# ai-forever/Kandinsky-2

Measured on NVIDIA H100. Metric: unet_denoising_steps_per_sec, higher is better.
Workload: dtype f16

## Files before the change

kandinsky-2_b200/csrc/k2_api.cu:

```cuda
#include <stdio.h>
#include <stdlib.h>
#include <string.h>

#include <algorithm>
#include <atomic>
#include <mutex>

#include "../../include/k2b200.h"
#include "k2_internal.h"

namespace k2 {

static thread_local std::string g_err;
static std::atomic<long long> g_launches{0};
static int g_force_bn = 0;
static int g_force_split = 0;
static int g_pdl = 0;


void set_error(const std::string& msg) { g_err = msg; }
int fail(const std::string& msg) {
  g_err = msg;
  return -1;
}
void count_launch(int n) { g_launches.fetch_add(n, std::memory_order_relaxed); }

bool pdl_enabled() { return g_pdl != 0; }
static int g_conv_epi_sets = 1;
static int g_gn_bps = 0;
int gn_apply_blocks_per_sm() { return g_gn_bps; }

int num_sms() {
  static int n = 0;
  if (n == 0) {
    int dev = 0;
    cudaGetDevice(&dev);
    cudaDeviceGetAttribute(&n, cudaDevAttrMultiProcessorCount, dev);
    if (n <= 0) n = 132;
  }
  return n;
}

typedef CUresult (*EncodeTiledFn)(CUtensorMap*, CUtensorMapDataType, cuuint32_t, void*, const cuuint64_t*,
                                  const cuuint64_t*, const cuuint32_t*, const cuuint32_t*,
                                  CUtensorMapInterleave, CUtensorMapSwizzle, CUtensorMapL2promotion,
                                  CUtensorMapFloatOOBfill);

static EncodeTiledFn get_encode_fn() {
  static EncodeTiledFn fn = nullptr;
  static std::once_flag once;
  std::call_once(once, [] {
    void* p = nullptr;
    cudaDriverEntryPointQueryResult qres;
    cudaError_t e = cudaGetDriverEntryPoint("cuTensorMapEncodeTiled", &p, cudaEnableDefault, &qres);
    if (e == cudaSuccess && qres == cudaDriverEntryPointSuccess) fn = reinterpret_cast<EncodeTiledFn>(p);
  });
  return fn;
}

int encode_tmap_f16(CUtensorMap* out, const void* base, int rank, const uint64_t* dims,
                    const uint64_t* strides_bytes, const uint32_t* box) {
  EncodeTiledFn fn = get_encode_fn();
  if (!fn) return fail("cuTensorMapEncodeTiled unavailable (no CUDA driver)");
  cuuint64_t gdim[5];
  cuuint64_t gstr[4];
  cuuint32_t bx[5];
  cuuint32_t es[5];
  for (int i = 0; i < rank; ++i) {
    gdim[i] = dims[i];
    bx[i] = box[i];
    es[i] = 1;
  }
  for (int i = 0; i + 1 < rank; ++i) gstr[i] = strides_bytes[i];
  CUresult r = fn(out, CU_TENSOR_MAP_DATA_TYPE_FLOAT16, static_cast<cuuint32_t>(rank), const_cast<void*>(base),
                  gdim, gstr, bx, es, CU_TENSOR_MAP_INTERLEAVE_NONE, CU_TENSOR_MAP_SWIZZLE_128B,
                  CU_TENSOR_MAP_L2_PROMOTION_L2_256B, CU_TENSOR_MAP_FLOAT_OOB_FILL_NONE);
  if (r != CUDA_SUCCESS) {
    char buf[256];
    snprintf(buf, sizeof buf,
             "cuTensorMapEncodeTiled failed (%d): rank %d dims %llu %llu %llu %llu box %u %u %u %u base %p",
             static_cast<int>(r), rank, (unsigned long long)dims[0], (unsigned long long)(rank > 1 ? dims[1] : 0),
             (unsigned long long)(rank > 2 ? dims[2] : 0), (unsigned long long)(rank > 3 ? dims[3] : 0), box[0],
             rank > 1 ? box[1] : 0, rank > 2 ? box[2] : 0, rank > 3 ? box[3] : 0, base);
    return fail(buf);
  }
  return 0;
}

static void choose_tile(int NB, int H, int W, int& TN, int& TH, int& TW, bool single_image_only = false) {
  long long best_tiles[2] = {-1, -1};
  int bn[2] = {1, 1}, bw[2] = {1, 1}, bh[2] = {1, 1};
  const int wmax = W < 128 ? W : 128;
  for (int tw = 1; tw <= wmax; ++tw) {
    const long long tiles_w = (W + tw - 1) / tw;
    for (int tn = 1; tn <= NB && tn * tw <= 128; ++tn) {
      int thmax = 128 / (tw * tn);
      if (thmax > H) thmax = H;
      if (thmax < 1) continue;
      const long long tiles_h = (H + thmax - 1) / thmax;
      const int th = static_cast<int>((H + tiles_h - 1) / tiles_h);
      const long long tiles = tiles_h * tiles_w * ((NB + tn - 1) / tn);
      for (int k = (tn == 1 ? 0 : 1); k < 2; ++k) {
        bool better = best_tiles[k] < 0 || tiles < best_tiles[k];
        if (!better && tiles == best_tiles[k]) {
          if (tn != bn[k]) {
            better = tn < bn[k];
          } else {
            const int d_new = tw > th ? tw - th : th - tw;
            const int d_old = bw[k] > bh[k] ? bw[k] - bh[k] : bh[k] - bw[k];
            better = (d_new < d_old) || (d_new == d_old && tw > bw[k]);
          }
        }
        if (better) {
          best_tiles[k] = tiles;
          bn[k] = tn;
          bw[k] = tw;
          bh[k] = th;
        }
      }
    }
  }
  const int k = (!single_image_only && best_tiles[1] * 100 <= best_tiles[0] * 85) ? 1 : 0;
  TN = bn[k];
  TW = bw[k];
  TH = bh[k];
}


struct ConvPlan {
  int TN, TH, TW, tiles_w, tiles_h, tiles_n, m_tiles;
  int m_tiles_phase;
  int BN, splits;
  int fuse_stats, row_groups;
  int es;
};

static void plan_conv(int NB, int H, int W, bool any9, int kchunks, int Cout, int out_mode, bool has_workspace,
                      long long workspace_bytes, bool want_gn, ConvPlan& pl, const int* cfg = nullptr, bool up2 = false,
                      bool w_batched = false) {
  const int g_force_bn = (cfg && cfg[0]) ? cfg[0] : k2::g_force_bn;
  const int g_force_split = (cfg && cfg[2]) ? cfg[2] : k2::g_force_split;
  pl.es = (cfg && cfg[3]) ? cfg[3] : k2::g_conv_epi_sets;
  choose_tile(NB, H, W, pl.TN, pl.TH, pl.TW, w_batched);
  pl.tiles_w = (W + pl.TW - 1) / pl.TW;
  pl.tiles_h = (H + pl.TH - 1) / pl.TH;
  pl.tiles_n = (NB + pl.TN - 1) / pl.TN;
  pl.m_tiles = pl.tiles_w * pl.tiles_h * pl.tiles_n;
  pl.m_tiles_phase = pl.m_tiles;

  int BN = g_force_bn;
  int splits = 1;
  const long long M_total = static_cast<long long>(NB) * H * W;
  const bool can_split = !up2 && !w_batched && has_workspace && out_mode == 0 && Cout % 8 == 0;
  auto split_ok = [&](int sp) {
    if (sp == 1) return true;
    const int kps = (kchunks + sp - 1) / sp;
    return can_split && kps >= 8 && (sp - 1) * kps < kchunks &&
           static_cast<long long>(sp) * M_total * Cout * 4 <= workspace_bytes;
  };
  auto model = [&](int bn, int sp) {
    const long long nt = (Cout + bn - 1) / bn;
    const long long units = static_cast<long long>(pl.m_tiles) * nt * sp * (up2 ? 4 : 1);
    const long long slots = num_sms();
    const long long waves = (units + slots - 1) / slots;
    const long long kps = (kchunks + sp - 1) / sp;
    long long cost = waves * (kps * (4LL * bn + 60) + 2000);
    if (sp > 1) cost += 4000 + (static_cast<long long>(sp) + 1) * M_total * Cout * 4 / 1800;
    return cost;
  };
  if (BN == 0) {
    if (Cout <= 16) BN = 16;
    else if (Cout <= 64) BN = 64;
    else if (Cout <= 128) BN = 128;
    else BN = 0;
  }
  {
    const int cand[3] = {256, 192, 128};
    long long best = -1;
    int best_bn = BN ? BN : 256, best_sp = 1;
    for (int ci = 0; ci < 3; ++ci) {
      const int bn = BN ? BN : cand[ci];
      if (BN && ci > 0) break;
      for (int sp = 1; sp <= 8; ++sp) {
        if (g_force_split > 0 && sp != g_force_split) continue;
        if (!split_ok(sp)) continue;
        const long long c = model(bn, sp);
        if (best < 0 || c < best) {
          best = c;
          best_bn = bn;
          best_sp = sp;
        }
      }
    }
    BN = best_bn;
    splits = best_sp;
  }
  pl.BN = BN;
  pl.splits = splits;

  pl.fuse_stats = 0;
  pl.row_groups = 0;
  if (want_gn && out_mode == 0 && Cout % 8 == 0) {
    if (splits == 1 && BN >= 64 && Cout % 64 == 0 && (pl.TN == 1 || pl.TH * pl.TW == 16)) {
      pl.fuse_stats = 1;
      pl.row_groups = ((pl.TN == 1) ? pl.m_tiles : NB * pl.tiles_h * pl.tiles_w) * (up2 ? 4 : 1);
    } else if (splits > 1 && (static_cast<long long>(H) * W) % 16 == 0) {
      pl.fuse_stats = 2;
      pl.row_groups = static_cast<int>(M_total / 16);
    }
  }
}

static void plan_to_info(const ConvPlan& pl, int* info) {
  if (!info) return;
  info[0] = pl.BN; info[1] = 0;
  info[2] = pl.splits; info[3] = pl.m_tiles; info[4] = pl.TN;
  info[5] = pl.fuse_stats; info[6] = pl.row_groups;
}

}

using namespace k2;

extern "C" {

const char* k2_last_error(void) { return g_err.c_str(); }
int k2_version(void) { return 100; }
long long k2_launch_count(void) { return g_launches.load(); }
void k2_reset_launch_count(void) { g_launches.store(0); }
int k2_set_tuning(int key, int value) {
  if (key == 0) {
    g_force_bn = value;
    return 0;
  }
  if (key == 1) {
    g_force_split = value;
    return 0;
  }
  if (key == 2) {
    if (value == 2) return fail("k2_set_tuning: no CTA-pair conv kernel on sm_90");
    return 0;
  }
  if (key == 4) {
    g_pdl = value;
    return 0;
  }
  if (key == 10) {
    g_conv_epi_sets = (value == 2) ? 2 : 1;
    return 0;
  }
  if (key == 11) {
    g_gn_bps = value;
    return 0;
  }
  if (key == 9) {
    return 0;
  }

  return fail("k2_set_tuning: unknown key");
}

int k2_conv_gemm(const K2ConvSrc* srcs, int nsrc, int NB, int H, int W, const void* w_packed, int w_rows,
                 int Ktot, int ldw, int Cout, const float* bias, const void* residual, int ldr, void* out, int ldo,
                 int out_mode, void* workspace, long long workspace_bytes, float* gn_partial, int* info,
                 k2_stream_t stream) {
  return k2_conv_gemm_cfg(srcs, nsrc, NB, H, W, w_packed, w_rows, Ktot, ldw, Cout, bias, residual, ldr, out, ldo, out_mode,
                          workspace, workspace_bytes, gn_partial, info, nullptr, 0, stream);
}

int k2_conv_gemm_cfg(const K2ConvSrc* srcs, int nsrc, int NB, int H, int W, const void* w_packed, int w_rows,
                     int Ktot, int ldw, int Cout, const float* bias, const void* residual, int ldr, void* out, int ldo,
                     int out_mode, void* workspace, long long workspace_bytes, float* gn_partial, int* info,
                     const int* cfg, long long w_batch_stride, k2_stream_t stream) {
  K2_REQUIRE(w_batch_stride >= 0 && w_batch_stride % 8 == 0, "conv_gemm_cfg: w_batch_stride must be a multiple of 8 elements");
  K2_REQUIRE(out_mode == 0 || out_mode == 1, "conv_gemm: out_mode must be 0 (fp16 rows) or 1 (fp32 NCHW)");
  K2_REQUIRE(out_mode == 0 || residual == nullptr, "conv_gemm: out_mode 1 (fp32 NCHW) takes no residual");
  const bool w_batched = w_batch_stride > 0;
  if (cfg) {
    K2_REQUIRE(cfg[0] == 0 || cfg[0] == 16 || cfg[0] == 64 || cfg[0] == 128 || cfg[0] == 192 || cfg[0] == 256,
               "conv_gemm_cfg: N tile must be 0, 16, 64, 128, 192 or 256");
    K2_REQUIRE(cfg[1] >= 0 && cfg[1] <= 2 && cfg[2] >= 0 && cfg[2] <= 8 && cfg[3] >= 0 && cfg[3] <= 2,
               "conv_gemm_cfg: pair mode in 0..2, splits in 0..8, epilogue sets in 0..2");
    K2_REQUIRE(cfg[1] != 2, "conv_gemm_cfg: no CTA-pair conv kernel on sm_90");
  }
  K2_REQUIRE(nsrc >= 1 && nsrc <= 3, "conv_gemm: 1..3 sources");
  K2_REQUIRE((reinterpret_cast<uintptr_t>(gn_partial) & 7) == 0, "conv_gemm: gn_partial must be 8-byte aligned");
  K2_REQUIRE(NB > 0 && H > 0 && W > 0 && Cout > 0, "conv_gemm: bad geometry");
  K2_REQUIRE(w_rows >= Cout, "conv_gemm: w_rows < Cout");
  K2_REQUIRE(Ktot % 64 == 0, "conv_gemm: Ktot must be a multiple of 64");
  if (ldw == 0) ldw = Ktot;
  K2_REQUIRE(ldw >= Ktot && ldw % 8 == 0 && (reinterpret_cast<uintptr_t>(w_packed) & 15) == 0,
             "conv_gemm: weight row stride / alignment");
  ConvGemmParams p;
  memset(&p, 0, sizeof p);
  p.NB = NB;
  p.H = H;
  p.W = W;
  bool any9 = false;
  int kchunks = 0;
  const bool up2 = srcs[0].taps == 4;
  if (up2) {
    K2_REQUIRE(nsrc == 1 && out_mode == 0 && residual == nullptr && H % 2 == 0 && W % 2 == 0,
               "conv_gemm: a taps == 4 source (3x3 conv over its nearest-2x upsampling) must be the only source, with fp16 "
               "output, no residual and even output H, W");
    H /= 2;
    W /= 2;
    p.H = H;
    p.W = W;
  }
  for (int s = 0; s < nsrc; ++s) {
    const K2ConvSrc& src = srcs[s];
    K2_REQUIRE(src.taps == 9 || src.taps == 1 || (s == 0 && src.taps == 4), "conv_gemm: taps must be 9 or 1 (or 4: up2)");
    K2_REQUIRE(src.C > 0 && src.C % 8 == 0 && src.ld % 8 == 0 && src.ld >= src.C, "conv_gemm: bad source C/ld");
    K2_REQUIRE((reinterpret_cast<uintptr_t>(src.ptr) & 15) == 0, "conv_gemm: source not 16B aligned");
    any9 = any9 || src.taps == 9;
    p.seg_taps[s] = src.taps;
    p.seg_kchunks[s] = (src.C + 63) / 64;
    kchunks += src.taps * p.seg_kchunks[s];
  }
  K2_REQUIRE(kchunks * 64 * (up2 ? 4 : 1) == Ktot,
             "conv_gemm: Ktot does not match the sources (taps * ceil(C/64)*64 summed; x4 phases for a taps == 4 source)");
  p.num_k_chunks = kchunks;

  ConvPlan pl;
  plan_conv(NB, H, W, any9 || up2, kchunks, Cout, out_mode, workspace != nullptr, workspace_bytes, gn_partial != nullptr, pl,
            cfg, up2, w_batched);
  K2_REQUIRE(!w_batched || (!up2 && pl.TN == 1), "conv_gemm_cfg: batched weights need single-image tiles");
  p.w_batched = w_batched ? 1 : 0;
  plan_to_info(pl, info);
  p.TN = pl.TN;
  p.TH = pl.TH;
  p.TW = pl.TW;
  p.tiles_w = pl.tiles_w;
  p.tiles_h = pl.tiles_h;
  p.tiles_n = pl.tiles_n;
  p.m_tiles = up2 ? 4 * pl.m_tiles_phase : pl.m_tiles;
  p.m_tiles_phase = pl.m_tiles_phase;
  p.up2 = up2 ? 1 : 0;
  p.a_box_bytes = static_cast<uint32_t>(p.TN * p.TH * p.TW * 128);
  for (int s = 0; s < nsrc; ++s) {
    const K2ConvSrc& src = srcs[s];
    uint64_t dims[4] = {static_cast<uint64_t>(src.C), static_cast<uint64_t>(W), static_cast<uint64_t>(H),
                        static_cast<uint64_t>(NB)};
    uint64_t str[3] = {static_cast<uint64_t>(src.ld) * 2, static_cast<uint64_t>(src.ld) * 2 * W,
                       static_cast<uint64_t>(src.ld) * 2 * W * H};
    uint32_t box[4] = {64, static_cast<uint32_t>(p.TW), static_cast<uint32_t>(p.TH), static_cast<uint32_t>(p.TN)};
    if (encode_tmap_f16(&p.tmA[s], src.ptr, 4, dims, str, box)) return -1;
  }
  const int BN = pl.BN, splits = pl.splits, fuse_stats = pl.fuse_stats;
  p.splits = splits;
  p.k_per_split = (kchunks + splits - 1) / splits;
  p.M_total = static_cast<long long>(NB) * H * W * (up2 ? 4 : 1);
  p.ws = reinterpret_cast<float*>(workspace);
  p.n_tiles = (Cout + BN - 1) / BN;
  p.Cout = Cout;
  {
    uint64_t dims[3] = {static_cast<uint64_t>(Ktot), static_cast<uint64_t>(w_rows), static_cast<uint64_t>(w_batched ? NB : 1)};
    uint64_t str[2] = {static_cast<uint64_t>(ldw) * 2,
                       (w_batched ? static_cast<uint64_t>(w_batch_stride) : static_cast<uint64_t>(ldw) * w_rows) * 2};
    uint32_t box[3] = {64, static_cast<uint32_t>(BN), 1};
    if (encode_tmap_f16(&p.tmB, w_packed, 3, dims, str, box)) return -1;
  }
  p.bias = bias;
  p.residual = reinterpret_cast<const __half*>(residual);
  p.ldr = ldr;
  p.out = out;
  p.ldo = ldo;
  p.out_mode = (splits > 1) ? 2 : out_mode;
  p.gn_part = (fuse_stats == 1) ? reinterpret_cast<float2*>(gn_partial) : nullptr;
  p.gn_mode = (fuse_stats == 1) ? (p.TN == 1 ? 1 : 2) : 0;
  if (out_mode == 0) {
    K2_REQUIRE(ldo % 8 == 0 && (reinterpret_cast<uintptr_t>(out) & 15) == 0, "conv_gemm: out alignment");
    if (residual)
      K2_REQUIRE(ldr % 8 == 0 && (reinterpret_cast<uintptr_t>(residual) & 15) == 0, "conv_gemm: residual alignment");
  }
  int rc = launch_conv_gemm(p, BN, pl.es, static_cast<cudaStream_t>(stream));
  if (rc == 0) g_launches.fetch_add(1, std::memory_order_relaxed);
  if (rc == 0 && splits > 1) {
    rc = launch_splitk_finalize(p.ws, splits, p.M_total, Cout, bias, p.residual, ldr, reinterpret_cast<__half*>(out), ldo,
                                fuse_stats == 2 ? reinterpret_cast<float2*>(gn_partial) : nullptr,
                                static_cast<cudaStream_t>(stream));
    if (rc == 0) g_launches.fetch_add(1, std::memory_order_relaxed);
  }
  return rc;
}

int k2_conv_plan(int NB, int H, int W, int taps, int Ktot, int Cout, int out_mode, long long workspace_bytes,
                 int want_gn_partial, int* info) {
  K2_REQUIRE(NB > 0 && H > 0 && W > 0 && Cout > 0 && info, "conv_plan: bad arguments");
  K2_REQUIRE(Ktot > 0 && Ktot % 64 == 0, "conv_plan: Ktot must be a positive multiple of 64");
  ConvPlan pl;
  plan_conv(NB, H, W, taps == 9, Ktot / 64, Cout, out_mode, workspace_bytes > 0, workspace_bytes, want_gn_partial != 0, pl);
  plan_to_info(pl, info);
  return 0;
}

}
```

kandinsky-2_b200/csrc/k2_common.cuh:

```cuda
#pragma once
#include <cuda.h>
#include <cuda_fp16.h>
#include <cuda_runtime.h>
#include <stdint.h>
#include <stdio.h>

namespace k2 {

__device__ __forceinline__ uint32_t smem_u32(const void* p) {
  return static_cast<uint32_t>(__cvta_generic_to_shared(p));
}

__device__ __forceinline__ uint32_t lane_id() { return threadIdx.x & 31; }

__device__ __forceinline__ bool elect_one() {
  uint32_t pred = 0;
  asm volatile(
      "{\n"
      ".reg .b32 rx;\n"
      ".reg .pred px;\n"
      "elect.sync rx|px, 0xffffffff;\n"
      "selp.b32 %0, 1, 0, px;\n"
      "}\n"
      : "=r"(pred));
  return pred != 0;
}

__device__ __forceinline__ void mbar_init(uint64_t* bar, uint32_t count) {
  asm volatile("mbarrier.init.shared::cta.b64 [%0], %1;" ::"r"(smem_u32(bar)), "r"(count));
}
__device__ __forceinline__ void fence_barrier_init() {
  asm volatile("fence.mbarrier_init.release.cluster;" ::: "memory");
}
__device__ __forceinline__ void mbar_arrive_expect_tx(uint64_t* bar, uint32_t bytes) {
  asm volatile("mbarrier.arrive.expect_tx.shared::cta.b64 _, [%0], %1;" ::"r"(smem_u32(bar)),
               "r"(bytes)
               : "memory");
}
__device__ __forceinline__ void mbar_arrive(uint64_t* bar) {
  asm volatile("mbarrier.arrive.shared::cta.b64 _, [%0];" ::"r"(smem_u32(bar)) : "memory");
}
__device__ __forceinline__ bool mbar_try_wait(uint64_t* bar, uint32_t parity) {
  uint32_t ok;
  asm volatile(
      "{\n"
      ".reg .pred p;\n"
      "mbarrier.try_wait.parity.shared::cta.b64 p, [%1], %2;\n"
      "selp.b32 %0, 1, 0, p;\n"
      "}\n"
      : "=r"(ok)
      : "r"(smem_u32(bar)), "r"(parity)
      : "memory");
  return ok != 0;
}
__device__ __forceinline__ void mbar_wait(uint64_t* bar, uint32_t parity) {
  if (mbar_try_wait(bar, parity)) return;
  long long t0 = clock64();
  while (!mbar_try_wait(bar, parity)) {
    if (clock64() - t0 > 4000000000LL) {
      printf("k2b200: mbarrier wait timeout (block %d,%d,%d thread %d)\n", blockIdx.x, blockIdx.y,
             blockIdx.z, threadIdx.x);
      __trap();
    }
  }
}

__device__ __forceinline__ void mbar_wait_lean(uint64_t* bar, uint32_t parity) {
  if (mbar_try_wait(bar, parity)) return;
  long long t0 = clock64();
  while (!mbar_try_wait(bar, parity)) {
    if (clock64() - t0 > 4000000000LL) __trap();
  }
}

__device__ __forceinline__ void fence_proxy_async_smem() {
  asm volatile("fence.proxy.async.shared::cta;" ::: "memory");
}

__device__ __forceinline__ void tma_prefetch_desc(const CUtensorMap* tm) {
  asm volatile("prefetch.tensormap [%0];" ::"l"(reinterpret_cast<uint64_t>(tm)) : "memory");
}
__device__ __forceinline__ void tma_load_2d(void* dst, const CUtensorMap* tm, uint64_t* bar, int c0,
                                            int c1) {
  asm volatile(
      "cp.async.bulk.tensor.2d.shared::cluster.global.mbarrier::complete_tx::bytes [%0], [%1, {%3, "
      "%4}], [%2];"
      ::"r"(smem_u32(dst)),
      "l"(reinterpret_cast<uint64_t>(tm)), "r"(smem_u32(bar)), "r"(c0), "r"(c1)
      : "memory");
}
__device__ __forceinline__ void tma_load_3d(void* dst, const CUtensorMap* tm, uint64_t* bar, int c0,
                                            int c1, int c2) {
  asm volatile(
      "cp.async.bulk.tensor.3d.shared::cluster.global.mbarrier::complete_tx::bytes [%0], [%1, {%3, "
      "%4, %5}], [%2];"
      ::"r"(smem_u32(dst)),
      "l"(reinterpret_cast<uint64_t>(tm)), "r"(smem_u32(bar)), "r"(c0), "r"(c1), "r"(c2)
      : "memory");
}
__device__ __forceinline__ void tma_load_4d(void* dst, const CUtensorMap* tm, uint64_t* bar, int c0,
                                            int c1, int c2, int c3) {
  asm volatile(
      "cp.async.bulk.tensor.4d.shared::cluster.global.mbarrier::complete_tx::bytes [%0], [%1, {%3, "
      "%4, %5, %6}], [%2];"
      ::"r"(smem_u32(dst)),
      "l"(reinterpret_cast<uint64_t>(tm)), "r"(smem_u32(bar)), "r"(c0), "r"(c1), "r"(c2), "r"(c3)
      : "memory");
}

__device__ __forceinline__ uint64_t make_wgmma_desc(uint32_t smem_addr) {
  uint64_t d = 0;
  d |= static_cast<uint64_t>((smem_addr & 0x3FFFF) >> 4);
  d |= static_cast<uint64_t>(1) << 16;
  d |= static_cast<uint64_t>(1024 >> 4) << 32;
  d |= static_cast<uint64_t>(1) << 62;
  return d;
}
__device__ __forceinline__ void wgmma_fence() { asm volatile("wgmma.fence.sync.aligned;" ::: "memory"); }
__device__ __forceinline__ void wgmma_commit() { asm volatile("wgmma.commit_group.sync.aligned;" ::: "memory"); }
template <int N>
__device__ __forceinline__ void wgmma_wait() {
  asm volatile("wgmma.wait_group.sync.aligned %0;" ::"n"(N) : "memory");
}
__device__ __forceinline__ void wgmma_m64n16k16(float (&d)[8], uint64_t adesc, uint64_t bdesc, uint32_t accumulate) {
  asm volatile(
      "{\n"
      ".reg .pred p;\n"
      "setp.ne.b32 p, %10, 0;\n"
      "wgmma.mma_async.sync.aligned.m64n16k16.f32.f16.f16 "
      "{%0, %1, %2, %3, %4, %5, %6, %7}, %8, %9, p, 1, 1, 0, 0;\n"
      "}\n"
      : "+f"(d[0]), "+f"(d[1]), "+f"(d[2]), "+f"(d[3]), "+f"(d[4]), "+f"(d[5]), "+f"(d[6]), "+f"(d[7])
      : "l"(adesc), "l"(bdesc), "r"(accumulate));
}

__device__ __forceinline__ void wgmma_m64n64k16(float (&d)[32], uint64_t adesc, uint64_t bdesc, uint32_t accumulate) {
  asm volatile(
      "{\n"
      ".reg .pred p;\n"
      "setp.ne.b32 p, %34, 0;\n"
      "wgmma.mma_async.sync.aligned.m64n64k16.f32.f16.f16 "
      "{%0, %1, %2, %3, %4, %5, %6, %7, %8, %9, %10, %11, %12, %13, %14, %15, %16, %17, %18, %19, %20, %21, %22, %23, %24, %25, %26, %27, %28, %29, %30, %31}, %32, %33, p, 1, 1, 0, 0;\n"
      "}\n"
      : "+f"(d[0]), "+f"(d[1]), "+f"(d[2]), "+f"(d[3]), "+f"(d[4]), "+f"(d[5]), "+f"(d[6]), "+f"(d[7]), "+f"(d[8]), "+f"(d[9]), "+f"(d[10]), "+f"(d[11]), "+f"(d[12]), "+f"(d[13]), "+f"(d[14]), "+f"(d[15]), "+f"(d[16]), "+f"(d[17]), "+f"(d[18]), "+f"(d[19]), "+f"(d[20]), "+f"(d[21]), "+f"(d[22]), "+f"(d[23]), "+f"(d[24]), "+f"(d[25]), "+f"(d[26]), "+f"(d[27]), "+f"(d[28]), "+f"(d[29]), "+f"(d[30]), "+f"(d[31])
      : "l"(adesc), "l"(bdesc), "r"(accumulate));
}

#define K2_WGMMA_D8(o)                                                                                                  \
  "+f"(d[(o)]), "+f"(d[(o) + 1]), "+f"(d[(o) + 2]), "+f"(d[(o) + 3]), "+f"(d[(o) + 4]), "+f"(d[(o) + 5]), "+f"(d[(o) + 6]), \
      "+f"(d[(o) + 7])
#define K2_WGMMA_D32(o) K2_WGMMA_D8(o), K2_WGMMA_D8((o) + 8), K2_WGMMA_D8((o) + 16), K2_WGMMA_D8((o) + 24)

__device__ __forceinline__ void wgmma_m64n128k16(float (&d)[64], uint64_t adesc, uint64_t bdesc, uint32_t accumulate) {
  asm volatile(
      "{\n"
      ".reg .pred p;\n"
      "setp.ne.b32 p, %66, 0;\n"
      "wgmma.mma_async.sync.aligned.m64n128k16.f32.f16.f16 {"
      "%0, %1, %2, %3, %4, %5, %6, %7, %8, %9, %10, %11, %12, %13, %14, %15, "
      "%16, %17, %18, %19, %20, %21, %22, %23, %24, %25, %26, %27, %28, %29, %30, %31, "
      "%32, %33, %34, %35, %36, %37, %38, %39, %40, %41, %42, %43, %44, %45, %46, %47, "
      "%48, %49, %50, %51, %52, %53, %54, %55, %56, %57, %58, %59, %60, %61, %62, %63"
      "}, %64, %65, p, 1, 1, 0, 0;\n"
      "}\n"
      : K2_WGMMA_D32(0), K2_WGMMA_D32(32)
      : "l"(adesc), "l"(bdesc), "r"(accumulate));
}

__device__ __forceinline__ void wgmma_m64n192k16(float (&d)[96], uint64_t adesc, uint64_t bdesc, uint32_t accumulate) {
  asm volatile(
      "{\n"
      ".reg .pred p;\n"
      "setp.ne.b32 p, %98, 0;\n"
      "wgmma.mma_async.sync.aligned.m64n192k16.f32.f16.f16 {"
      "%0, %1, %2, %3, %4, %5, %6, %7, %8, %9, %10, %11, %12, %13, %14, %15, "
      "%16, %17, %18, %19, %20, %21, %22, %23, %24, %25, %26, %27, %28, %29, %30, %31, "
      "%32, %33, %34, %35, %36, %37, %38, %39, %40, %41, %42, %43, %44, %45, %46, %47, "
      "%48, %49, %50, %51, %52, %53, %54, %55, %56, %57, %58, %59, %60, %61, %62, %63, "
      "%64, %65, %66, %67, %68, %69, %70, %71, %72, %73, %74, %75, %76, %77, %78, %79, "
      "%80, %81, %82, %83, %84, %85, %86, %87, %88, %89, %90, %91, %92, %93, %94, %95"
      "}, %96, %97, p, 1, 1, 0, 0;\n"
      "}\n"
      : K2_WGMMA_D32(0), K2_WGMMA_D32(32), K2_WGMMA_D32(64)
      : "l"(adesc), "l"(bdesc), "r"(accumulate));
}

__device__ __forceinline__ void wgmma_m64n256k16(float (&d)[128], uint64_t adesc, uint64_t bdesc, uint32_t accumulate) {
  asm volatile(
      "{\n"
      ".reg .pred p;\n"
      "setp.ne.b32 p, %130, 0;\n"
      "wgmma.mma_async.sync.aligned.m64n256k16.f32.f16.f16 {"
      "%0, %1, %2, %3, %4, %5, %6, %7, %8, %9, %10, %11, %12, %13, %14, %15, "
      "%16, %17, %18, %19, %20, %21, %22, %23, %24, %25, %26, %27, %28, %29, %30, %31, "
      "%32, %33, %34, %35, %36, %37, %38, %39, %40, %41, %42, %43, %44, %45, %46, %47, "
      "%48, %49, %50, %51, %52, %53, %54, %55, %56, %57, %58, %59, %60, %61, %62, %63, "
      "%64, %65, %66, %67, %68, %69, %70, %71, %72, %73, %74, %75, %76, %77, %78, %79, "
      "%80, %81, %82, %83, %84, %85, %86, %87, %88, %89, %90, %91, %92, %93, %94, %95, "
      "%96, %97, %98, %99, %100, %101, %102, %103, %104, %105, %106, %107, %108, %109, %110, %111, "
      "%112, %113, %114, %115, %116, %117, %118, %119, %120, %121, %122, %123, %124, %125, %126, %127"
      "}, %128, %129, p, 1, 1, 0, 0;\n"
      "}\n"
      : K2_WGMMA_D32(0), K2_WGMMA_D32(32), K2_WGMMA_D32(64), K2_WGMMA_D32(96)
      : "l"(adesc), "l"(bdesc), "r"(accumulate));
}
__device__ __forceinline__ uint64_t make_wgmma_desc_mn(uint32_t smem_addr) {
  uint64_t d = 0;
  d |= static_cast<uint64_t>((smem_addr & 0x3FFFF) >> 4);
  d |= static_cast<uint64_t>(1) << 16;
  d |= static_cast<uint64_t>(1024 >> 4) << 32;
  d |= static_cast<uint64_t>(1) << 62;
  return d;
}

__device__ __forceinline__ void wgmma_m64n64k16_rs_tb(float (&d)[32], const uint32_t (&a)[4], uint64_t bdesc) {
  asm volatile(
      "{\n"
      "wgmma.mma_async.sync.aligned.m64n64k16.f32.f16.f16 {"
      "%0, %1, %2, %3, %4, %5, %6, %7, %8, %9, %10, %11, %12, %13, %14, %15, "
      "%16, %17, %18, %19, %20, %21, %22, %23, %24, %25, %26, %27, %28, %29, %30, %31"
      "}, {%32, %33, %34, %35}, %36, 1, 1, 1, 1;\n"
      "}\n"
      : K2_WGMMA_D32(0)
      : "r"(a[0]), "r"(a[1]), "r"(a[2]), "r"(a[3]), "l"(bdesc));
}
#undef K2_WGMMA_D32
#undef K2_WGMMA_D8

__device__ __forceinline__ void reg_fence(float& r) { asm volatile("" : "+f"(r)::"memory"); }

template <int R>
__device__ __forceinline__ void setmaxnreg_dec() {
  asm volatile("setmaxnreg.dec.sync.aligned.u32 %0;" ::"n"(R));
}
template <int R>
__device__ __forceinline__ void setmaxnreg_inc() {
  asm volatile("setmaxnreg.inc.sync.aligned.u32 %0;" ::"n"(R));
}

__device__ __forceinline__ void mma_16816(float (&d)[4], const uint32_t (&a)[4], uint32_t b0, uint32_t b1) {
  asm volatile(
      "mma.sync.aligned.m16n8k16.row.col.f32.f16.f16.f32 {%0, %1, %2, %3}, {%4, %5, %6, %7}, {%8, %9}, "
      "{%0, %1, %2, %3};"
      : "+f"(d[0]), "+f"(d[1]), "+f"(d[2]), "+f"(d[3])
      : "r"(a[0]), "r"(a[1]), "r"(a[2]), "r"(a[3]), "r"(b0), "r"(b1));
}
__device__ __forceinline__ void ldmatrix_x4(uint32_t (&r)[4], uint32_t saddr) {
  asm volatile("ldmatrix.sync.aligned.m8n8.x4.shared.b16 {%0, %1, %2, %3}, [%4];"
               : "=r"(r[0]), "=r"(r[1]), "=r"(r[2]), "=r"(r[3])
               : "r"(saddr));
}
__device__ __forceinline__ void ldmatrix_x4_trans(uint32_t (&r)[4], uint32_t saddr) {
  asm volatile("ldmatrix.sync.aligned.m8n8.x4.trans.shared.b16 {%0, %1, %2, %3}, [%4];"
               : "=r"(r[0]), "=r"(r[1]), "=r"(r[2]), "=r"(r[3])
               : "r"(saddr));
}
__device__ __forceinline__ void cp_async_16(uint32_t saddr, const void* gptr, int src_bytes) {
  asm volatile("cp.async.cg.shared.global [%0], [%1], 16, %2;" ::"r"(saddr), "l"(gptr), "r"(src_bytes) : "memory");
}
__device__ __forceinline__ void cp_async_commit() { asm volatile("cp.async.commit_group;" ::: "memory"); }
template <int N>
__device__ __forceinline__ void cp_async_wait() {
  asm volatile("cp.async.wait_group %0;" ::"n"(N) : "memory");
}

__device__ __forceinline__ void sts_v4(uint32_t saddr, uint32_t a, uint32_t b, uint32_t c, uint32_t d) {
  asm volatile("st.shared.v4.b32 [%0], {%1, %2, %3, %4};" ::"r"(saddr), "r"(a), "r"(b), "r"(c), "r"(d) : "memory");
}
__device__ __forceinline__ uint4 lds_v4(uint32_t saddr) {
  uint4 v;
  asm volatile("ld.shared.v4.b32 {%0, %1, %2, %3}, [%4];" : "=r"(v.x), "=r"(v.y), "=r"(v.z), "=r"(v.w) : "r"(saddr) : "memory");
  return v;
}
__device__ __forceinline__ uint32_t lds_u32(uint32_t saddr) {
  uint32_t v;
  asm volatile("ld.shared.b32 %0, [%1];" : "=r"(v) : "r"(saddr) : "memory");
  return v;
}
__device__ __forceinline__ void named_bar_sync(int id, int count) {
  asm volatile("bar.sync %0, %1;" ::"r"(id), "r"(count) : "memory");
}
__device__ __forceinline__ void named_bar_arrive(int id, int count) {
  asm volatile("bar.arrive %0, %1;" ::"r"(id), "r"(count) : "memory");
}
__device__ __forceinline__ void pdl_wait() { asm volatile("griddepcontrol.wait;" ::: "memory"); }
__device__ __forceinline__ void pdl_launch() { asm volatile("griddepcontrol.launch_dependents;" ::: "memory"); }

__device__ __forceinline__ float silu_f(float x) {
  float e, r;
  asm("ex2.approx.ftz.f32 %0, %1;" : "=f"(e) : "f"(-1.44269504088896341f * x));
  asm("rcp.approx.ftz.f32 %0, %1;" : "=f"(r) : "f"(1.f + e));
  return x * r;
}

}
```

kandinsky-2_b200/csrc/k2_conv_gemm.cu:

```cuda
#include <stdio.h>

#include "k2_common.cuh"
#include "k2_internal.h"

namespace k2 {

namespace {

constexpr int BM = 128;
constexpr int BK = 64;
constexpr int A_STAGE_BYTES = BM * BK * 2;
constexpr int ACC_PAD = 4;

constexpr int EPI_STAGE_FLOATS = 32 * 33;
constexpr int EPI_BYTES = 4 * EPI_STAGE_FLOATS * 4 + 4 * 256 * 4;
constexpr int SMEM_LIMIT = 227 * 1024;

template <int BN, int ES>
struct Cfg {
  static constexpr int B_STAGE_BYTES = BN * BK * 2;
  static constexpr int STAGE_BYTES = A_STAGE_BYTES + B_STAGE_BYTES;
  static constexpr int BNC = (BN < 64) ? BN : (ES == 2 ? 128 : 64);
  static_assert(ES == 1 || BN % 128 == 0, "two epilogue sets need N tiles of 128 or 256");
  static constexpr int ACC_BYTES = BM * (BNC + ACC_PAD) * 4;
  static constexpr int BAR_BYTES = 256;
  static constexpr int FIXED = ACC_BYTES + ES * EPI_BYTES + BAR_BYTES + 1024;
  static constexpr int STAGES = (SMEM_LIMIT - FIXED) / STAGE_BYTES > 6 ? 6 : (SMEM_LIMIT - FIXED) / STAGE_BYTES;
  static constexpr int SMEM_BYTES = STAGES * STAGE_BYTES + FIXED;
  static_assert(STAGES >= 2, "conv_gemm: shared memory does not hold two pipeline stages");
};

__device__ __forceinline__ void decode_m_tile(const ConvGemmParams& p, int m_idx, int& n0, int& y0,
                                              int& x0, int& phase) {
  phase = 0;
  if (p.up2) {
    phase = m_idx / p.m_tiles_phase;
    m_idx -= phase * p.m_tiles_phase;
  }
  int tw_i = m_idx % p.tiles_w;
  int t = m_idx / p.tiles_w;
  int th_i = t % p.tiles_h;
  int tn_i = t / p.tiles_h;
  x0 = tw_i * p.TW;
  y0 = th_i * p.TH;
  n0 = tn_i * p.TN;
}

template <int N>
__device__ __forceinline__ void acc_ld(const float* src, uint32_t (&r)[N]) {
#pragma unroll
  for (int v = 0; v < N / 4; ++v) {
    const float4 t = *reinterpret_cast<const float4*>(src + 4 * v);
    r[4 * v] = __float_as_uint(t.x);
    r[4 * v + 1] = __float_as_uint(t.y);
    r[4 * v + 2] = __float_as_uint(t.z);
    r[4 * v + 3] = __float_as_uint(t.w);
  }
}

template <int BN, int ES>
__device__ __forceinline__ void epilogue_tile(const ConvGemmParams& p, const float* acc, int ew, int lane, int n0, int y0,
                                              int x0, int cbase, int split, int m_idx, float* stat_smem, int es_arg,
                                              int phase) {
  const int es = (ES == 1) ? 0 : es_arg;
  const int row = ew * 32 + lane;
  const int thw = p.TH * p.TW;
  constexpr int CH = (BN >= 32) ? 32 : 16;
  const float* arow = acc + row * (BN + ACC_PAD);
      const int tn = row / thw;
      const int rem = row - tn * thw;
      const int th = rem / p.TW;
      const int tw = rem - th * p.TW;
      const int n = n0 + tn, y = y0 + th, x = x0 + tw;
      const bool valid = (tn < p.TN) && (n < p.NB) && (y < p.H) && (x < p.W);
      const long long out_row = p.up2 ? (static_cast<long long>(n) * (2 * p.H) + (2 * y + (phase >> 1))) * (2 * p.W) + (2 * x + (phase & 1))
                                      : (static_cast<long long>(n) * p.H + y) * p.W + x;
      const int m_in = p.up2 ? m_idx - phase * p.m_tiles_phase : m_idx;
      auto part_index = [&](long long base) { return p.up2 ? base * 4 + phase : base; };
      if constexpr (BN % 64 == 0) {
        if ((p.out_mode == 0 && p.Cout % 64 == 0) || (p.out_mode == 2 && p.Cout % 32 == 0)) {
          const uint32_t stage = smem_u32(stat_smem + (es * 4 + ew) * EPI_STAGE_FLOATS);
          float* bsm = stat_smem + 4 * ES * EPI_STAGE_FLOATS + (es * 4 + ew) * 256;
          const int my_pix = valid ? static_cast<int>(out_row) : -1;
          const int sub = lane >> 3, piece = lane & 7;
          int pix[8];
#pragma unroll
          for (int i = 0; i < 8; ++i) pix[i] = __shfl_sync(0xffffffffu, my_pix, i * 4 + sub);
          const uint32_t own = stage + lane * 128;
          if (p.out_mode == 2) {
            float* wsb = p.ws + static_cast<long long>(split) * p.M_total * p.Cout;
#pragma unroll 1
            for (int j = 0; j < BN / 32; ++j) {
              const int col0 = cbase + j * 32;
              if (col0 >= p.Cout) break;
              if constexpr (ES > 1) {
                if ((j % ES) != es) continue;
              }
              uint32_t r[32];
              acc_ld(arow + j * 32, r);
#pragma unroll
              for (int v = 0; v < 8; ++v)
                sts_v4(own + ((v ^ (lane & 7)) << 4), r[v * 4], r[v * 4 + 1], r[v * 4 + 2], r[v * 4 + 3]);
              __syncwarp();
#pragma unroll
              for (int i = 0; i < 8; ++i) {
                const int rr = i * 4 + sub;
                const uint4 v4 = lds_v4(stage + rr * 128 + ((piece ^ (rr & 7)) << 4));
                if (pix[i] >= 0)
                  *reinterpret_cast<uint4*>(wsb + static_cast<long long>(pix[i]) * p.Cout + col0 + piece * 4) = v4;
              }
              __syncwarp();
            }
            return;
          }
          constexpr int NP = BN / 64;
          if (p.bias) {
#pragma unroll
            for (int c = lane; c < BN; c += 32) bsm[c] = (cbase + c < p.Cout) ? __ldg(p.bias + cbase + c) : 0.f;
            __syncwarp();
          }
          __half* outb = reinterpret_cast<__half*>(p.out);
          float4 st[NP];
          uint4 rpre[8];
          auto load_res = [&](int jp) {
            const int c0 = cbase + jp * 64;
#pragma unroll
            for (int i = 0; i < 8; ++i) {
              rpre[i] = make_uint4(0u, 0u, 0u, 0u);
              if (pix[i] >= 0 && c0 < p.Cout)
                rpre[i] = *reinterpret_cast<const uint4*>(p.residual + static_cast<long long>(pix[i]) * p.ldr + c0 + piece * 8);
            }
          };
          if constexpr (ES == 1) {
            if (p.residual) load_res(0);
          }
#pragma unroll
          for (int jp = 0; jp < NP; ++jp) {
            const int col0 = cbase + jp * 64;
            st[jp] = make_float4(0.f, 0.f, 0.f, 0.f);
            if (col0 < p.Cout && (ES == 1 || (jp % ES) == es)) {
              if constexpr (ES > 1) {
                if (p.residual) load_res(jp);
              }
              if (p.residual) {
#pragma unroll
                for (int i = 0; i < 8; ++i) {
                  const int rr = i * 4 + sub;
                  sts_v4(stage + rr * 128 + ((piece ^ (rr & 7)) << 4), rpre[i].x, rpre[i].y, rpre[i].z, rpre[i].w);
                }
                __syncwarp();
              }
              if constexpr (ES == 1) {
                if (p.residual && jp + 1 < NP) load_res(jp + 1);
              }
#pragma unroll
              for (int v = 0; v < 8; ++v) {
                uint32_t r[8];
                acc_ld(arow + jp * 64 + v * 8, r);
                float f[8];
#pragma unroll
                for (int e = 0; e < 8; ++e) f[e] = __uint_as_float(r[e]);
                if (p.bias) {
                  const float4 b0 = *reinterpret_cast<const float4*>(bsm + jp * 64 + v * 8);
                  const float4 b1 = *reinterpret_cast<const float4*>(bsm + jp * 64 + v * 8 + 4);
                  f[0] += b0.x; f[1] += b0.y; f[2] += b0.z; f[3] += b0.w;
                  f[4] += b1.x; f[5] += b1.y; f[6] += b1.z; f[7] += b1.w;
                }
                const uint32_t slot = own + ((v ^ (lane & 7)) << 4);
                if (p.residual) {
                  const uint4 rv = lds_v4(slot);
                  const __half2* rh = reinterpret_cast<const __half2*>(&rv);
#pragma unroll
                  for (int e = 0; e < 4; ++e) {
                    const float2 t = __half22float2(rh[e]);
                    f[2 * e] += t.x;
                    f[2 * e + 1] += t.y;
                  }
                }
                uint32_t o[4];
#pragma unroll
                for (int e = 0; e < 4; ++e) {
                  const __half2 hh = __floats2half2_rn(f[2 * e], f[2 * e + 1]);
                  o[e] = valid ? *reinterpret_cast<const uint32_t*>(&hh) : 0u;
                }
                sts_v4(slot, o[0], o[1], o[2], o[3]);
              }
              __syncwarp();
#pragma unroll
              for (int i = 0; i < 8; ++i) {
                const int rr = i * 4 + sub;
                const uint4 v4 = lds_v4(stage + rr * 128 + ((piece ^ (rr & 7)) << 4));
                if (pix[i] >= 0)
                  *reinterpret_cast<uint4*>(outb + static_cast<long long>(pix[i]) * p.ldo + col0 + piece * 8) = v4;
              }
              if (p.gn_part) {
                float4 h0 = make_float4(0.f, 0.f, 0.f, 0.f), h1 = make_float4(0.f, 0.f, 0.f, 0.f);
#pragma unroll
                for (int rr = 0; rr < 32; ++rr) {
                  const uint32_t w = lds_u32(stage + rr * 128 + (((lane >> 2) ^ (rr & 7)) << 4) + ((lane & 3) << 2));
                  const float2 t = __half22float2(*reinterpret_cast<const __half2*>(&w));
                  float4& hacc = (rr < 16) ? h0 : h1;
                  hacc.x += t.x;
                  hacc.y = fmaf(t.x, t.x, hacc.y);
                  hacc.z += t.y;
                  hacc.w = fmaf(t.y, t.y, hacc.w);
                }
                if (p.gn_mode == 2) {
                  const int per = p.tiles_h * p.tiles_w;
                  const int sp = m_in % per;
                  const int img = n0 + 2 * ew;
                  if (2 * ew < p.TN && img < p.NB)
                    *reinterpret_cast<float4*>(p.gn_part + part_index(static_cast<long long>(img) * per + sp) * p.Cout + col0 + 2 * lane) = h0;
                  if (2 * ew + 1 < p.TN && img + 1 < p.NB)
                    *reinterpret_cast<float4*>(p.gn_part + part_index(static_cast<long long>(img + 1) * per + sp) * p.Cout + col0 + 2 * lane) = h1;
                } else {
                  st[jp] = make_float4(h0.x + h1.x, h0.y + h1.y, h0.z + h1.z, h0.w + h1.w);
                }
              }
              __syncwarp();
            }
          }
          if (p.gn_part && p.gn_mode == 1) {
            if constexpr (ES == 1) {
              float4* mine = reinterpret_cast<float4*>(stat_smem + ew * EPI_STAGE_FLOATS);
#pragma unroll
              for (int jp = 0; jp < NP; ++jp) mine[jp * 32 + lane] = st[jp];
              named_bar_sync(1, 128);
              if (ew < NP) {
                const int col0 = cbase + ew * 64;
                if (col0 < p.Cout) {
                  float4 acc = make_float4(0.f, 0.f, 0.f, 0.f);
#pragma unroll
                  for (int w = 0; w < 4; ++w) {
                    const float4 t = reinterpret_cast<const float4*>(stat_smem + w * EPI_STAGE_FLOATS)[ew * 32 + lane];
                    acc.x += t.x; acc.y += t.y; acc.z += t.z; acc.w += t.w;
                  }
                  *reinterpret_cast<float4*>(p.gn_part + part_index(m_in) * p.Cout + col0 + 2 * lane) = acc;
                }
              }
              named_bar_sync(1, 128);
            } else {
              float4* mine = reinterpret_cast<float4*>(stat_smem + (es * 4 + ew) * EPI_STAGE_FLOATS);
#pragma unroll
              for (int jp = 0; jp < NP; ++jp) mine[jp * 32 + lane] = st[jp];
              named_bar_sync(1 + es, 128);
              const int jp_f = es + ew * ES;
              if (jp_f < NP) {
                const int col0 = cbase + jp_f * 64;
                if (col0 < p.Cout) {
                  float4 acc = make_float4(0.f, 0.f, 0.f, 0.f);
#pragma unroll
                  for (int w = 0; w < 4; ++w) {
                    const float4 t =
                        reinterpret_cast<const float4*>(stat_smem + (es * 4 + w) * EPI_STAGE_FLOATS)[jp_f * 32 + lane];
                    acc.x += t.x; acc.y += t.y; acc.z += t.z; acc.w += t.w;
                  }
                  *reinterpret_cast<float4*>(p.gn_part + part_index(m_in) * p.Cout + col0 + 2 * lane) = acc;
                }
              }
              named_bar_sync(1 + es, 128);
            }
          }
          return;
        }
      }
#pragma unroll 1
      for (int j = 0; j < BN / CH; ++j) {
        uint32_t r[CH];
        acc_ld(arow + j * CH, r);
        const int col0 = cbase + j * CH;
        if (valid && col0 < p.Cout) {
          if (p.out_mode == 2) {
            float* w = p.ws + (static_cast<long long>(split) * p.M_total + out_row) * p.Cout + col0;
            if (col0 + CH <= p.Cout) {
#pragma unroll
              for (int v = 0; v < CH / 4; ++v)
                *reinterpret_cast<uint4*>(w + v * 4) = make_uint4(r[v * 4], r[v * 4 + 1], r[v * 4 + 2], r[v * 4 + 3]);
            } else {
#pragma unroll
              for (int e = 0; e < CH; ++e)
                if (col0 + e < p.Cout) w[e] = __uint_as_float(r[e]);
            }
          } else if (p.out_mode == 0) {
            __half* orow = reinterpret_cast<__half*>(p.out) + out_row * p.ldo + col0;
            const __half* rrow = p.residual ? p.residual + out_row * p.ldr + col0 : nullptr;
            if (col0 + CH <= p.Cout) {
#pragma unroll
              for (int v = 0; v < CH / 8; ++v) {
                float f[8];
#pragma unroll
                for (int e = 0; e < 8; ++e) {
                  f[e] = __uint_as_float(r[v * 8 + e]);
                  if (p.bias) f[e] += __ldg(p.bias + col0 + v * 8 + e);
                }
                if (rrow) {
                  uint4 rv = *reinterpret_cast<const uint4*>(rrow + v * 8);
                  const __half2* rh = reinterpret_cast<const __half2*>(&rv);
#pragma unroll
                  for (int e = 0; e < 4; ++e) {
                    float2 t = __half22float2(rh[e]);
                    f[2 * e] += t.x;
                    f[2 * e + 1] += t.y;
                  }
                }
                uint4 ov;
                __half2* oh = reinterpret_cast<__half2*>(&ov);
#pragma unroll
                for (int e = 0; e < 4; ++e) oh[e] = __floats2half2_rn(f[2 * e], f[2 * e + 1]);
                *reinterpret_cast<uint4*>(orow + v * 8) = ov;
              }
            } else {
#pragma unroll
              for (int e = 0; e < CH; ++e) {
                if (col0 + e < p.Cout) {
                  float f = __uint_as_float(r[e]);
                  if (p.bias) f += __ldg(p.bias + col0 + e);
                  if (rrow) f += __half2float(rrow[e]);
                  orow[e] = __float2half_rn(f);
                }
              }
            }
          } else {
            float* o = reinterpret_cast<float*>(p.out);
#pragma unroll
            for (int e = 0; e < CH; ++e) {
              if (col0 + e < p.Cout) {
                float f = __uint_as_float(r[e]);
                if (p.bias) f += __ldg(p.bias + col0 + e);
                o[((static_cast<long long>(n) * p.Cout + (col0 + e)) * p.H + y) * p.W + x] = f;
              }
            }
          }
        }
      }
}


template <int BN, int ES>
__global__ void __launch_bounds__(384, 1) conv_gemm_kernel(const __grid_constant__ ConvGemmParams p) {
  using C = Cfg<BN, ES>;
  constexpr int BNC = C::BNC;
  constexpr int NA = BN / 2;
  extern __shared__ uint8_t smem_raw[];
  uint8_t* smem = reinterpret_cast<uint8_t*>((reinterpret_cast<uintptr_t>(smem_raw) + 1023) &
                                             ~static_cast<uintptr_t>(1023));
  float* acc_smem = reinterpret_cast<float*>(smem + C::STAGES * C::STAGE_BYTES);
  float* stat_smem = reinterpret_cast<float*>(smem + C::STAGES * C::STAGE_BYTES + C::ACC_BYTES);
  uint64_t* full_bar = reinterpret_cast<uint64_t*>(smem + C::STAGES * C::STAGE_BYTES + C::ACC_BYTES + ES * EPI_BYTES);
  uint64_t* empty_bar = full_bar + C::STAGES;

  const int warp_idx = threadIdx.x >> 5;
  const int lane = threadIdx.x & 31;
  const int wg = warp_idx >> 2;

  if (threadIdx.x == 0) {
    tma_prefetch_desc(&p.tmB);
    for (int s = 0; s < 3; ++s)
      if (p.seg_taps[s]) tma_prefetch_desc(&p.tmA[s]);
    for (int i = 0; i < C::STAGES; ++i) {
      mbar_init(&full_bar[i], 1);
      mbar_init(&empty_bar[i], 8);
    }
    fence_barrier_init();
  }
  __syncthreads();
  pdl_wait();
  pdl_launch();

  const int total_tiles = p.m_tiles * p.n_tiles * p.splits;

  if (wg == 0) {
    setmaxnreg_dec<40>();
    if (warp_idx == 0 && elect_one()) {
      int stage = 0;
      uint32_t ring_phase = 0;
      const uint32_t tx_bytes = p.a_box_bytes + C::B_STAGE_BYTES;
      for (int tile = blockIdx.x; tile < total_tiles; tile += gridDim.x) {
        const int n_idx = tile % p.n_tiles;
        const int m_idx = (tile / p.n_tiles) % p.m_tiles;
        const int split = tile / (p.m_tiles * p.n_tiles);
        int n0, y0, x0, phase;
        decode_m_tile(p, m_idx, n0, y0, x0, phase);
        const int kb = phase * p.num_k_chunks;
        const int k0 = split * p.k_per_split;
        const int k1 = min(p.num_k_chunks, k0 + p.k_per_split);
        int s = 0, rem = k0;
        while (rem >= p.seg_taps[s] * p.seg_kchunks[s]) {
          rem -= p.seg_taps[s] * p.seg_kchunks[s];
          ++s;
        }
        int tap = rem / p.seg_kchunks[s];
        int c = rem - tap * p.seg_kchunks[s];
        for (int kc = k0; kc < k1; ++kc) {
          const int taps = p.seg_taps[s];
          const int dy = (taps == 9) ? (tap / 3 - 1) : (taps == 4 ? (tap >> 1) + (phase >> 1) - 1 : 0);
          const int dx = (taps == 9) ? (tap % 3 - 1) : (taps == 4 ? (tap & 1) + (phase & 1) - 1 : 0);
          mbar_wait_lean(&empty_bar[stage], ring_phase ^ 1);
          uint8_t* sA = smem + stage * C::STAGE_BYTES;
          uint8_t* sB = sA + A_STAGE_BYTES;
          mbar_arrive_expect_tx(&full_bar[stage], tx_bytes);
          tma_load_4d(sA, &p.tmA[s], &full_bar[stage], c * BK, x0 + dx, y0 + dy, n0);
          tma_load_3d(sB, &p.tmB, &full_bar[stage], (kb + kc) * BK, n_idx * BN, p.w_batched ? n0 : 0);
          if (++stage == C::STAGES) {
            stage = 0;
            ring_phase ^= 1;
          }
          if (++c == p.seg_kchunks[s]) {
            c = 0;
            if (++tap == taps) {
              tap = 0;
              ++s;
            }
          }
        }
      }
    }
  } else {
    setmaxnreg_inc<232>();
    const int g = wg - 1;
    const int w = warp_idx & 3;
    int stage = 0;
    uint32_t phase = 0;
    for (int tile = blockIdx.x; tile < total_tiles; tile += gridDim.x) {
      const int n_idx = tile % p.n_tiles;
      const int m_idx = (tile / p.n_tiles) % p.m_tiles;
      const int split = tile / (p.m_tiles * p.n_tiles);
      const int nk = min(p.num_k_chunks, (split + 1) * p.k_per_split) - split * p.k_per_split;
      float acc[NA];
#pragma unroll
      for (int i = 0; i < NA; ++i) acc[i] = 0.f;
      int prev_stage = -1;
      for (int kc = 0; kc < nk; ++kc) {
        mbar_wait_lean(&full_bar[stage], phase);
        const uint32_t a_addr = smem_u32(smem + stage * C::STAGE_BYTES) + g * (64 * 128);
        const uint32_t b_addr = smem_u32(smem + stage * C::STAGE_BYTES + A_STAGE_BYTES);
        wgmma_fence();
#pragma unroll
        for (int k = 0; k < BK / 16; ++k) {
          const uint64_t adesc = make_wgmma_desc(a_addr) + static_cast<uint64_t>(k * 2);
          const uint64_t bdesc = make_wgmma_desc(b_addr) + static_cast<uint64_t>(k * 2);
          if constexpr (BN == 256) {
            wgmma_m64n256k16(acc, adesc, bdesc, 1u);
          } else if constexpr (BN == 192) {
            wgmma_m64n192k16(acc, adesc, bdesc, 1u);
          } else if constexpr (BN == 128) {
            wgmma_m64n128k16(acc, adesc, bdesc, 1u);
          } else if constexpr (BN == 64) {
            wgmma_m64n64k16(acc, adesc, bdesc, 1u);
          } else {
            static_assert(BN == 16, "conv_gemm: N tile without a wgmma shape");
            wgmma_m64n16k16(acc, adesc, bdesc, 1u);
          }
        }
        wgmma_commit();
        wgmma_wait<1>();
        if (prev_stage >= 0 && lane == 0) mbar_arrive(&empty_bar[prev_stage]);
        prev_stage = stage;
        if (++stage == C::STAGES) {
          stage = 0;
          phase ^= 1;
        }
      }
      wgmma_wait<0>();
      if (prev_stage >= 0 && lane == 0) mbar_arrive(&empty_bar[prev_stage]);

      int n0, y0, x0, mphase;
      decode_m_tile(p, m_idx, n0, y0, x0, mphase);
      const int r0 = 64 * g + 16 * w + (lane >> 2);
      const int cq = 2 * (lane & 3);
#pragma unroll
      for (int pass = 0; pass < BN / BNC; ++pass) {
        named_bar_sync(3, 256);
#pragma unroll
        for (int i = 0; i < NA; i += 2) {
          if ((8 * (i >> 2)) / BNC != pass) continue;
          const int row = r0 + 8 * ((i >> 1) & 1);
          const int col = 8 * (i >> 2) - pass * BNC + cq;
          *reinterpret_cast<float2*>(acc_smem + row * (BNC + ACC_PAD) + col) = make_float2(acc[i], acc[i + 1]);
        }
        named_bar_sync(3, 256);
        if (ES == 2 || g == 0)
          epilogue_tile<BNC, ES>(p, acc_smem, w, lane, n0, y0, x0, n_idx * BN + pass * BNC, split, m_idx, stat_smem, g,
                                 mphase);
      }
    }
  }
}

__global__ void __launch_bounds__(256) splitk_finalize_kernel(const float* __restrict__ ws, int splits, long long M,
                                                              int Cout, const float* __restrict__ bias,
                                                              const __half* __restrict__ residual, int ldr,
                                                              __half* __restrict__ out, int ldo, float2* __restrict__ gn_part) {
  __shared__ float red[8][32][17];
  const int vx = threadIdx.x & 31, ry = threadIdx.x >> 5;
  const int c0 = (blockIdx.y * 32 + vx) * 8;
  const long long rg = blockIdx.x;
  pdl_wait();
  pdl_launch();
  float st[16];
#pragma unroll
  for (int e = 0; e < 16; ++e) st[e] = 0.f;
  if (c0 < Cout) {
    float bv[8];
#pragma unroll
    for (int e = 0; e < 8; ++e) bv[e] = bias ? __ldg(bias + c0 + e) : 0.f;
#pragma unroll
    for (int rr = 0; rr < 2; ++rr) {
      const long long m = rg * 16 + ry + rr * 8;
      if (m >= M) continue;
      float f[8];
#pragma unroll
      for (int e = 0; e < 8; ++e) f[e] = bv[e];
      for (int s = 0; s < splits; ++s) {
        const float4* w = reinterpret_cast<const float4*>(ws + (static_cast<long long>(s) * M + m) * Cout + c0);
        const float4 a = __ldcs(w), b = __ldcs(w + 1);
        f[0] += a.x; f[1] += a.y; f[2] += a.z; f[3] += a.w; f[4] += b.x; f[5] += b.y; f[6] += b.z; f[7] += b.w;
      }
      if (residual) {
        const uint4 rv = __ldg(reinterpret_cast<const uint4*>(residual + m * ldr + c0));
        const __half2* rh = reinterpret_cast<const __half2*>(&rv);
#pragma unroll
        for (int e = 0; e < 4; ++e) {
          const float2 t = __half22float2(rh[e]);
          f[2 * e] += t.x;
          f[2 * e + 1] += t.y;
        }
      }
      uint4 ov;
      __half2* oh = reinterpret_cast<__half2*>(&ov);
#pragma unroll
      for (int e = 0; e < 4; ++e) {
        oh[e] = __floats2half2_rn(f[2 * e], f[2 * e + 1]);
        const float2 t = __half22float2(oh[e]);
        st[2 * e] += t.x;
        st[2 * e + 1] += t.y;
        st[8 + 2 * e] = fmaf(t.x, t.x, st[8 + 2 * e]);
        st[8 + 2 * e + 1] = fmaf(t.y, t.y, st[8 + 2 * e + 1]);
      }
      *reinterpret_cast<uint4*>(out + m * ldo + c0) = ov;
    }
  }
  if (gn_part == nullptr) return;
#pragma unroll
  for (int e = 0; e < 16; ++e) red[ry][vx][e] = st[e];
  __syncthreads();
  const int vx2 = threadIdx.x >> 3, e2 = threadIdx.x & 7;
  const int c = (blockIdx.y * 32 + vx2) * 8 + e2;
  if (c < Cout) {
    float s1 = 0.f, s2 = 0.f;
#pragma unroll
    for (int q = 0; q < 8; ++q) {
      s1 += red[q][vx2][e2];
      s2 += red[q][vx2][8 + e2];
    }
    gn_part[rg * Cout + c] = make_float2(s1, s2);
  }
}


template <int BN, int ES>
int launch_bn(const ConvGemmParams& p, cudaStream_t stream) {
  using C = Cfg<BN, ES>;
  static bool attr_set = false;
  if (!attr_set) {
    K2_CHECK_CUDA(cudaFuncSetAttribute(conv_gemm_kernel<BN, ES>, cudaFuncAttributeMaxDynamicSharedMemorySize,
                                       C::SMEM_BYTES));
    attr_set = true;
  }
  int total = p.m_tiles * p.n_tiles * p.splits;
  int grid = total < num_sms() ? total : num_sms();
  K2_CHECK_CUDA(launch_k(conv_gemm_kernel<BN, ES>, dim3(grid), dim3(384), C::SMEM_BYTES, stream, p));
  return 0;
}

}

int launch_splitk_finalize(const float* ws, int splits, long long M, int Cout, const float* bias, const __half* residual,
                           int ldr, __half* out, int ldo, float2* gn_part, cudaStream_t stream) {
  dim3 grid(static_cast<unsigned int>((M + 15) / 16), (Cout / 8 + 31) / 32);
  K2_CHECK_CUDA(launch_k(splitk_finalize_kernel, grid, dim3(256), 0, stream, ws, splits, M, Cout, bias, residual, ldr, out, ldo,
                         gn_part));
  return 0;
}

int launch_conv_gemm(const ConvGemmParams& p, int BN, int epilogue_sets, cudaStream_t stream) {
  if (epilogue_sets == 2) {
    switch (BN) {
      case 128: return launch_bn<128, 2>(p, stream);
      case 256: return launch_bn<256, 2>(p, stream);
      default: break;
    }
  }
  switch (BN) {
    case 16: return launch_bn<16, 1>(p, stream);
    case 64: return launch_bn<64, 1>(p, stream);
    case 128: return launch_bn<128, 1>(p, stream);
    case 192: return launch_bn<192, 1>(p, stream);
    case 256: return launch_bn<256, 1>(p, stream);
    default: return fail("conv_gemm: unsupported BN");
  }
}

}
```

kandinsky-2_b200/csrc/k2_internal.h:

```cpp
#pragma once
#include <cuda.h>
#include <cuda_fp16.h>
#include <cuda_runtime.h>
#include <stdint.h>

#include <string>

namespace k2 {

void set_error(const std::string& msg);
int fail(const std::string& msg);
#define K2_CHECK_CUDA(expr)                                                                 \
  do {                                                                                      \
    cudaError_t _e = (expr);                                                                \
    if (_e != cudaSuccess)                                                                  \
      return ::k2::fail(std::string(#expr) + ": " + cudaGetErrorString(_e));                \
  } while (0)
#define K2_REQUIRE(cond, msg)                                  \
  do {                                                         \
    if (!(cond)) return ::k2::fail(std::string("k2b200: ") + (msg)); \
  } while (0)

inline bool aligned16(const void* p) { return (reinterpret_cast<uintptr_t>(p) & 15) == 0; }

int num_sms();
bool pdl_enabled();

template <typename... KArgs, typename... Args>
inline cudaError_t launch_k(void (*kernel)(KArgs...), dim3 grid, dim3 block, size_t smem, cudaStream_t stream,
                            Args&&... args) {
  cudaLaunchConfig_t cfg = {};
  cfg.gridDim = grid;
  cfg.blockDim = block;
  cfg.dynamicSmemBytes = smem;
  cfg.stream = stream;
  cudaLaunchAttribute attr[1];
  attr[0].id = cudaLaunchAttributeProgrammaticStreamSerialization;
  attr[0].val.programmaticStreamSerializationAllowed = 1;
  cfg.attrs = attr;
  cfg.numAttrs = pdl_enabled() ? 1 : 0;
  return cudaLaunchKernelEx(&cfg, kernel, static_cast<KArgs>(args)...);
}
void count_launch(int n = 1);

int encode_tmap_f16(CUtensorMap* out, const void* base, int rank, const uint64_t* dims,
                    const uint64_t* strides_bytes , const uint32_t* box);

struct ConvGemmParams {
  CUtensorMap tmA[3];
  CUtensorMap tmB;
  int w_batched;
  int seg_taps[3];
  int seg_kchunks[3];
  int num_k_chunks;
  int NB, H, W;
  int TN, TH, TW;
  int tiles_n, tiles_h, tiles_w;
  int m_tiles, n_tiles;
  int Cout;
  const float* bias;
  const __half* residual;
  int ldr;
  void* out;
  int ldo;
  int out_mode;
  uint32_t a_box_bytes;
  int splits;
  int k_per_split;
  float* ws;
  long long M_total;
  float2* gn_part;
  int gn_mode;
  int up2;
  int m_tiles_phase;
};
int launch_conv_gemm(const ConvGemmParams& p, int BN, int epilogue_sets, cudaStream_t stream);
int launch_splitk_finalize(const float* ws, int splits, long long M, int Cout, const float* bias, const __half* residual,
                           int ldr, __half* out, int ldo, float2* gn_part, cudaStream_t stream);

struct FlashParams {
  const __half* qkv;
  long long ldq;
  int hs, q_off, k_off, v_off;
  const __half* enc;
  long long lde;
  int ehs, ek_off, ev_off;
  int B, heads, T, Tc;
  __half* out;
  int ldo, ohs;
  float scale_log2e;
};
int gn_apply_blocks_per_sm();
int launch_attention(const FlashParams& p, int head_dim, cudaStream_t stream);

}
```

kandinsky-2_b200/kandinsky2/launch_plan.py:

```python
import gc
import os

import torch

from . import ops

FOLD_MAX_RG = int(os.environ.get("K2_GN_FOLD_MAX_RG", "18"))
TUNE = os.environ.get("K2_AUTOTUNE", "1") != "0"
FORK = os.environ.get("K2_FORK", "1") != "0"
TUNE_SMALL_M = int(os.environ.get("K2_TUNE_SMALL_M", "8192"))
_tune_cache = {}


def tune(key, run, m_rows=0):
    if not TUNE:
        return None
    key = (torch.cuda.current_device(), TUNE_SMALL_M) + key
    if key in _tune_cache:
        return _tune_cache[key]
    info = [0] * 7
    run(None, info)
    bn0, splits = info[0], info[2]
    cout = key[3]
    best = None
    if cout > 64:
        bns = [bn0] if splits > 1 else [bn for bn in (128, 192, 256) if bn - 64 < cout or bn == bn0]
        cands = [(bn0, 0, splits, 1)] + [(bn, 0, splits, es) for bn in bns for es in ((1,) if bn == 192 else (1, 2))
                                        if (bn, es) != (bn0, 1)]
        if 0 < m_rows <= TUNE_SMALL_M and splits == 1:
            for bn in (128, 192, 256):
                if bn - 64 >= cout:
                    continue
                for sp in (2, 3, 4):
                    probe = [0] * 7
                    try:
                        run((bn, 1, sp, 1), probe)
                    except Exception:
                        continue
                    if probe[0] == bn and probe[2] == sp:
                        cands.append((bn, 1, sp, 1))

        def timed(cfg, reps=6):
            run(cfg)
            evs = [torch.cuda.Event(enable_timing=True) for _ in range(reps + 1)]
            evs[0].record()
            for i in range(reps):
                run(cfg)
                evs[i + 1].record()
            torch.cuda.synchronize()
            return min(evs[i].elapsed_time(evs[i + 1]) for i in range(reps))

        t0 = tb = timed(cands[0])
        for cfg in cands[1:]:
            t = timed(cfg)
            if t < tb and t < 0.97 * t0:
                t = max(t, timed(cfg))
                if t < tb and t < 0.97 * t0:
                    best, tb = cfg, t
    _tune_cache[key] = best
    return best


class LaunchPlan:
    def __init__(self, dev, nb):
        self.dev = dev
        self.NB = nb
        self._parts = {}
        self._scratch = {}
        self.steps = []
        self.graph = None
        self._side_stream = None
        self._side_open = False
        self._serial = False

    def _tmp(self, slot, *shape, dtype=torch.float16):
        key = (slot, dtype) + tuple(shape)
        if key not in self._scratch:
            self._scratch[key] = torch.empty(*shape, device=self.dev, dtype=dtype)
        return self._scratch[key]

    def _new(self, *shape, dtype=torch.float16):
        return torch.empty(*shape, device=self.dev, dtype=dtype)

    def _add(self, fn, kind="misc", flops=0):
        fn()
        self.steps.append((fn, kind, flops))

    def _side(self, fn, kind="misc", flops=0):
        if not FORK:
            return self._add(fn, kind, flops)
        first = not self._side_open
        self._side_open = True

        def step():
            if self._serial:
                return fn()
            if self._side_stream is None:
                self._side_stream = torch.cuda.Stream(device=self.dev)
            if first:
                ev = torch.cuda.Event()
                ev.record()
                self._side_stream.wait_event(ev)
            with torch.cuda.stream(self._side_stream):
                fn()
        self._add(step, kind, flops)

    def _join(self):
        if not self._side_open:
            return
        self._side_open = False

        def step():
            if self._serial:
                return
            ev = torch.cuda.Event()
            ev.record(self._side_stream)
            torch.cuda.current_stream().wait_event(ev)
        self._add(step, "join", 0)

    def _conv(self, srcs, w, cout, out, flops, bias=None, residual=None, want_stats=True, part_slot=None, out_mode=0,
              geom=None, w_batch_stride=0, kind="conv_gemm"):
        part = None
        if want_stats and out_mode == 0:
            g = geom if geom is not None else tuple(out.shape[:3])
            n = ops.gn_part_floats(g[0], g[1], g[2], cout)
            part = self._tmp(part_slot, n, dtype=torch.float32) if part_slot else self._new(n, dtype=torch.float32)
        info = [0] * 7
        run = lambda cfg, info=None: ops.conv_gemm(srcs, w, cout, bias=bias, residual=residual, out=out, gn_part=part,
                                                   info=info, cfg=cfg, out_mode=out_mode, geom=geom,
                                                   w_batch_stride=w_batch_stride)
        key = ("conv", cout, tuple(out.shape), geom, tuple((t.shape[-1], taps) for t, taps in srcs), residual is not None,
               part is not None, out_mode, w_batch_stride > 0)
        cfg = tune(key, run, m_rows=out.shape[0] * out.shape[1] * out.shape[2] if out_mode == 0 and geom is None else 0)
        self._add(lambda: run(cfg, info), kind, flops)
        if part is not None and info[5]:
            self._parts[out.data_ptr()] = (part, info[6] // (geom[0] if geom is not None else out.shape[0]))
        else:
            self._parts.pop(out.data_ptr(), None)

    def _gemm(self, x, w, cout, out, flops, bias=None, residual=None):
        run = lambda cfg, info=None: ops.gemm_rows(x, w, cout, bias=bias, residual=residual, out=out, cfg=cfg, info=info)
        cfg = tune(("gemm", cout, tuple(x.shape), residual is not None), run, m_rows=x.shape[0] * x.shape[1])
        self._add(lambda: run(cfg), "conv_gemm", flops)
        self._parts.pop(out.data_ptr(), None)

    def _stats(self, a, b, eps):
        pa = self._parts.get(a.data_ptr())
        pb = self._parts.get(b.data_ptr()) if b is not None else None
        st = self._new(self.NB, 32, 2, dtype=torch.float32)
        HW = a.shape[1] * a.shape[2]
        if pa is not None and (b is None or pb is not None):
            c1 = b.shape[-1] if b is not None else 0
            self._add(lambda: ops.gn_finalize(pa[0], a.shape[-1], pb[0] if pb else None, c1, self.NB, pa[1], HW, st,
                                              rg1=pb[1] if pb else None, eps=eps), "gn_finalize")
        else:
            self._add(lambda: ops.gn_stats(a, b, stats=st, eps=eps), "gn_stats")
        return st

    def _norm(self, a, b, gamma, beta, y, film=None, act=1, resample=0, xres=None, eps=1e-5):
        pa = self._parts.get(a.data_ptr())
        pb = self._parts.get(b.data_ptr()) if b is not None else None
        have = pa is not None and (b is None or pb is not None)
        cpg = (a.shape[-1] + (b.shape[-1] if b is not None else 0)) // 32
        if have and cpg >= 2 and max(pa[1], pb[1] if pb else 0) <= FOLD_MAX_RG:
            self._add(lambda: ops.gn_apply_fold(a, b, pa[0], pa[1], pb[0] if pb else None, pb[1] if pb else 0, gamma, beta,
                                                film=film, act=act, resample=resample, y=y, xres=xres, eps=eps), "gn_apply")
            return
        st = self._stats(a, b, eps)
        self._add(lambda: ops.gn_apply(a, b, st, gamma, beta, film=film, act=act, resample=resample, y=y, xres=xres),
                  "gn_apply")

    def launch(self):
        for fn, _, _ in self.steps:
            fn()

    def _timed_pass(self):
        evs = []
        self._serial = True
        torch.cuda.synchronize()
        torch.cuda._sleep(int(4e7))
        for fn, kind, flops in self.steps:
            s = torch.cuda.Event(enable_timing=True)
            e = torch.cuda.Event(enable_timing=True)
            s.record()
            fn()
            e.record()
            evs.append((s, e))
        torch.cuda.synchronize()
        self._serial = False
        return [s.elapsed_time(e) for s, e in evs]

    def profile_detail(self, reps=3):
        acc = [0.0] * len(self.steps)
        for _ in range(reps):
            for i, ms in enumerate(self._timed_pass()):
                acc[i] += ms / reps
        return [(k, f, ms) for (_, k, f), ms in zip(self.steps, acc)]

    def profile(self, reps=3):
        agg = {}
        for kind, flops, ms in self.profile_detail(reps):
            if kind == "join":
                continue
            a = agg.setdefault(kind, dict(ms=0.0, launches=0, flops=0))
            a["ms"] += ms
            a["launches"] += 1
            a["flops"] += flops
        return agg

    def run(self, use_graph):
        if not use_graph:
            self.launch()
            return
        if self.graph is None:
            self.launch()
            torch.cuda.synchronize()
            self.graph = capture_graph(self.launch)
        self.graph.replay()


def capture_graph(launch):
    g = torch.cuda.CUDAGraph()
    enabled = gc.isenabled()
    gc.disable()
    try:
        with torch.cuda.graph(g):
            launch()
    finally:
        if enabled:
            gc.enable()
    return g
```

profiles/conv_layers.py:

```python
import argparse
import json
import os
import subprocess
import sys

ROOT = os.path.dirname(os.path.dirname(os.path.abspath(__file__)))
for p in (ROOT, os.path.join(ROOT, "kandinsky-2_b200")):
    if p not in sys.path:
        sys.path.insert(0, p)

import torch

B, H, W = 4, 96, 96


def _card():
    q = subprocess.run(["nvidia-smi", "--query-gpu=name,power.limit,clocks.max.sm", "--format=csv,noheader", "-i", "0"],
                       capture_output=True, text=True)
    return q.stdout.strip() or torch.cuda.get_device_name(0)


def _pad64(c):
    return (c + 63) // 64 * 64


def _layer(key, dev, g):
    from kandinsky2 import ops
    rnd = lambda *s: torch.randn(*s, device=dev, generator=g).half()
    kind, cout = key[0], key[1]
    if kind == "gemm":
        _, _, xshape, has_res = key
        x = rnd(*xshape)
        M, K = x.numel() // xshape[-1], xshape[-1]
        w = rnd(cout, K)
        bias = torch.randn(cout, device=dev, generator=g)
        res = rnd(*xshape[:-1], cout) if has_res else None
        out = torch.empty(*xshape[:-1], cout, device=dev, dtype=torch.float16)
        run = lambda cfg, info=None: ops.gemm_rows(x, w, cout, bias=bias, residual=res, out=out, cfg=cfg, info=info)
        return run, dict(M=M, N=cout, K=K, desc=f"gemm {M}x{K}->{cout}" + (" +res" if has_res else ""))
    _, _, oshape, geom, srcs_spec, has_res, has_part, out_mode, w_batched = key
    if w_batched:
        return None, None
    if geom is not None:
        NB, Ho, Wo = geom
    elif out_mode == 0:
        NB, Ho, Wo = oshape[:3]
    else:
        NB, Ho, Wo = oshape[0], oshape[2], oshape[3]
    up2 = srcs_spec[0][1] == 4
    Hs, Ws = (Ho // 2, Wo // 2) if up2 else (Ho, Wo)
    srcs = [(rnd(NB, Hs, Ws, c), taps) for c, taps in srcs_spec]
    K = sum(taps * _pad64(c) for c, taps in srcs_spec)
    w_rows = max(16, cout)
    w = rnd(w_rows, 4 * K if up2 else K)
    bias = torch.randn(cout, device=dev, generator=g)
    res = rnd(NB, Ho, Wo, cout) if has_res else None
    out = torch.empty(*oshape, device=dev, dtype=torch.float16 if out_mode == 0 else torch.float32)
    part = torch.zeros(ops.gn_part_floats(NB, Ho, Wo, cout), device=dev) if has_part else None
    run = lambda cfg, info=None: ops.conv_gemm(srcs, w, cout, bias=bias, residual=res, out=out, out_mode=out_mode, geom=geom,
                                               gn_part=part, cfg=cfg, info=info)
    desc = (f"{NB}x{Ho}x{Wo} " + "+".join(f"{c}{'x3x3' if t == 9 else ('up2' if t == 4 else 'x1x1')}" for c, t in srcs_spec)
            + f"->{cout}" + (" +res" if has_res else "") + (" fp32-nchw" if out_mode else ""))
    return run, dict(M=NB * Ho * Wo, N=cout, K=K, desc=desc)


def _time(run, cfg, min_ms):
    for _ in range(3):
        run(cfg)
    torch.cuda.synchronize()
    s, e = torch.cuda.Event(enable_timing=True), torch.cuda.Event(enable_timing=True)
    s.record()
    for _ in range(5):
        run(cfg)
    e.record()
    torch.cuda.synchronize()
    reps = max(10, int(min_ms / max(s.elapsed_time(e) / 5, 1e-3)) + 1)
    s.record()
    for _ in range(reps):
        run(cfg)
    e.record()
    torch.cuda.synchronize()
    return s.elapsed_time(e) / reps, reps


def main():
    ap = argparse.ArgumentParser()
    ap.add_argument("--out", default=None)
    ap.add_argument("--min-ms", type=float, default=50.0, help="timed window per configuration")
    ap.add_argument("--mma-n", default="tile", choices=["tile", "64"],
                    help="wgmma N of the build: one instruction per N tile, or m64n64k16 per 64 columns")
    args = ap.parse_args()
    if not torch.cuda.is_available():
        raise SystemExit("needs a CUDA sm_90 device")
    import bench
    from kandinsky2 import launch_plan, ops
    from kandinsky2.model.gaussian_diffusion import FusedStep, create_ddpm_v22
    dev = torch.device("cuda", 0)
    torch.cuda.set_device(dev)
    ops.set_tuning(4, 1)
    res = {"card": _card(), "torch": torch.__version__, "geometry": f"cfg-2: UNet batch {2 * B}, {H}x{W} latents",
           "mma_n": args.mma_n, "min_ms": args.min_ms}

    counts = {}
    tune = launch_plan.tune

    def counting_tune(key, run, m_rows=0):
        counts[key] = counts.get(key, 0) + 1
        return tune(key, run, m_rows=m_rows)
    launch_plan.tune = counting_tune
    model = bench.build_unet(dev)
    image_emb = torch.randn(2 * B, 1280, generator=torch.Generator().manual_seed(1234)).to(dev)
    step = FusedStep(model, B, H, W, dict(image_emb=image_emb), guidance_scale=4.0, cond_first=False, clip_range=2.0,
                     threshold_mode=0)
    launch_plan.tune = tune
    diffusion = create_ddpm_v22(50)
    coef, ts = diffusion._tables(dev)
    order = torch.arange(diffusion.num_timesteps - 1, -1, -1, device=dev)
    step.set_schedule(ts[order], coef[order], torch.randn(len(order), B, 4, H, W, device=dev))
    x = step.latent()
    x.copy_(torch.randn(B, 4, H, W, device=dev))
    step.advance(x)
    torch.cuda.synchronize()
    res["plan_conv_launches"] = sum(1 for _, kind, _ in step.plan.steps if kind == "conv_gemm")
    res["counted_conv_launches"] = sum(counts.values())

    g = torch.Generator(device=dev).manual_seed(7)
    layers = []
    for key, n in counts.items():
        run, shp = _layer(key, dev, g)
        if run is None:
            continue
        info = [0] * 7
        picked = launch_plan._tune_cache.get((dev.index, launch_plan.TUNE_SMALL_M) + key)
        run(picked, info)
        picked_cfg = [info[0], 0, info[2], (picked[3] if picked and picked[3] else 1)]
        cout = shp["N"]
        cfgs = []
        if cout > 64:
            cfgs = [(bn, 0, 1, es) for bn in (128, 192, 256) if bn - 64 < cout or bn == info[0]
                    for es in ((1,) if bn == 192 else (1, 2))]
        if tuple(picked_cfg) not in cfgs:
            cfgs.append(tuple(picked_cfg))
        rows = []
        for cfg in cfgs:
            info = [0] * 7
            run(cfg, info)
            bn, splits = info[0], info[2]
            ms, reps = _time(run, cfg, args.min_ms)
            flops = 2.0 * shp["M"] * cout * shp["K"]
            mma_n = bn if (args.mma_n == "tile" or bn < 64) else 64
            smem_bpf = (2048 + 32 * mma_n) / (2.0 * 64 * mma_n * 16)
            m_tiles = info[3] * (4 if "up2" in shp["desc"] else 1)
            chunks = m_tiles * ((cout + bn - 1) // bn) * (shp["K"] // 64)
            l2_bytes = chunks * (16384 + bn * 128)
            rows.append(dict(n_tile=bn, epilogue_sets=cfg[3], splits=splits, ms=round(ms, 5), reps=reps,
                             tflops=round(flops / (ms * 1e-3) / 1e12, 1),
                             smem_operand_bytes_per_flop=round(smem_bpf, 5),
                             l2_operand_bytes_per_flop=round(l2_bytes / flops, 5),
                             l2_operand_TBps=round(l2_bytes / (ms * 1e-3) / 1e12, 2)))
        pick = next((r for r in rows if [r["n_tile"], r["splits"], r["epilogue_sets"]] ==
                     [picked_cfg[0], picked_cfg[2], picked_cfg[3]]), rows[0])
        layers.append(dict(shape=shp["desc"], key=repr(key), launches_per_step=n, gemm_gflop=round(2e-9 * shp["M"] * cout * shp["K"], 3),
                           picked=dict(n_tile=picked_cfg[0], splits=picked_cfg[2], epilogue_sets=picked_cfg[3],
                                       tuned=picked is not None),
                           picked_ms=pick["ms"], configs=rows))
    total = sum(l["launches_per_step"] * l["picked_ms"] for l in layers)
    for l in layers:
        l["share_of_conv_time"] = round(l["launches_per_step"] * l["picked_ms"] / total, 4)
    layers.sort(key=lambda l: -l["share_of_conv_time"])
    res["conv_ms_per_step_at_picked"] = round(total, 3)
    res["layers"] = layers

    print(f"# {res['card']}  (mma_n={args.mma_n})  conv time per step at the picked configurations: {total:.2f} ms")
    print(f"{'shape':44s} {'n':>2s} {'share':>6s} {'pick':>9s}  " + "  ".join(f"{c:>9s}" for c in
          ("128/1", "128/2", "192/1", "256/1", "256/2")) + "   (TFLOP/s at N tile / epilogue sets, splits 1)")
    for l in layers:
        by = {(r["n_tile"], r["epilogue_sets"]): r["tflops"] for r in l["configs"] if r["splits"] == 1}
        pk = l["picked"]
        print(f"{l['shape'][:44]:44s} {l['launches_per_step']:2d} {100 * l['share_of_conv_time']:5.1f}% "
              f"{pk['n_tile']:>3d}/{pk['epilogue_sets']}/{pk['splits']:<3d}  " +
              "  ".join(f"{by.get(c, float('nan')):9.1f}" for c in ((128, 1), (128, 2), (192, 1), (256, 1), (256, 2))))
    if args.out:
        os.makedirs(os.path.dirname(os.path.abspath(args.out)), exist_ok=True)
        with open(args.out, "w") as f:
            f.write(json.dumps(res, indent=1) + "\n")


if __name__ == "__main__":
    main()
```

Before: 30.92.

## Run conv epilogue from registers via per-warp staging, drop shared accumulator buffer

Removes the shared-memory fp32 accumulator tile and the two-epilogue-set variant. Each math warp now stages its own register accumulators, adding bias and residual (residual prefetched with cp.async into swizzled per-warp blocks), and folds GroupNorm partials through a small fold buffer. The smaller fixed footprint lets more pipeline stages fit in shared memory, and static asserts now require a minimum stage count per N tile. The tuning path and the profiler drop the epilogue-set option. Risks are higher register pressure and a more complex per-warp epilogue.

```diff
diff --git a/kandinsky-2_b200/csrc/k2_api.cu b/kandinsky-2_b200/csrc/k2_api.cu
--- a/kandinsky-2_b200/csrc/k2_api.cu
+++ b/kandinsky-2_b200/csrc/k2_api.cu
@@ -26,7 +26,6 @@
 void count_launch(int n) { g_launches.fetch_add(n, std::memory_order_relaxed); }
 
 bool pdl_enabled() { return g_pdl != 0; }
-static int g_conv_epi_sets = 1;
 static int g_gn_bps = 0;
 int gn_apply_blocks_per_sm() { return g_gn_bps; }
 
@@ -132,7 +131,6 @@
   int m_tiles_phase;
   int BN, splits;
   int fuse_stats, row_groups;
-  int es;
 };
 
 static void plan_conv(int NB, int H, int W, bool any9, int kchunks, int Cout, int out_mode, bool has_workspace,
@@ -140,7 +138,6 @@
                       bool w_batched = false) {
   const int g_force_bn = (cfg && cfg[0]) ? cfg[0] : k2::g_force_bn;
   const int g_force_split = (cfg && cfg[2]) ? cfg[2] : k2::g_force_split;
-  pl.es = (cfg && cfg[3]) ? cfg[3] : k2::g_conv_epi_sets;
   choose_tile(NB, H, W, pl.TN, pl.TH, pl.TW, w_batched);
   pl.tiles_w = (W + pl.TW - 1) / pl.TW;
   pl.tiles_h = (H + pl.TH - 1) / pl.TH;
@@ -245,15 +242,14 @@
     g_pdl = value;
     return 0;
   }
-  if (key == 10) {
-    g_conv_epi_sets = (value == 2) ? 2 : 1;
-    return 0;
-  }
   if (key == 11) {
     g_gn_bps = value;
     return 0;
   }
   if (key == 9) {
+    return 0;
+  }
+  if (key == 10) {
     return 0;
   }
 
@@ -374,7 +370,7 @@
     if (residual)
       K2_REQUIRE(ldr % 8 == 0 && (reinterpret_cast<uintptr_t>(residual) & 15) == 0, "conv_gemm: residual alignment");
   }
-  int rc = launch_conv_gemm(p, BN, pl.es, static_cast<cudaStream_t>(stream));
+  int rc = launch_conv_gemm(p, BN, static_cast<cudaStream_t>(stream));
   if (rc == 0) g_launches.fetch_add(1, std::memory_order_relaxed);
   if (rc == 0 && splits > 1) {
     rc = launch_splitk_finalize(p.ws, splits, p.M_total, Cout, bias, p.residual, ldr, reinterpret_cast<__half*>(out), ldo,
diff --git a/kandinsky-2_b200/csrc/k2_common.cuh b/kandinsky-2_b200/csrc/k2_common.cuh
--- a/kandinsky-2_b200/csrc/k2_common.cuh
+++ b/kandinsky-2_b200/csrc/k2_common.cuh
@@ -267,6 +267,15 @@
 __device__ __forceinline__ void sts_v4(uint32_t saddr, uint32_t a, uint32_t b, uint32_t c, uint32_t d) {
   asm volatile("st.shared.v4.b32 [%0], {%1, %2, %3, %4};" ::"r"(saddr), "r"(a), "r"(b), "r"(c), "r"(d) : "memory");
 }
+__device__ __forceinline__ void sts_u32(uint32_t saddr, uint32_t a) {
+  asm volatile("st.shared.b32 [%0], %1;" ::"r"(saddr), "r"(a) : "memory");
+}
+__device__ __forceinline__ void sts_v2f(uint32_t saddr, float a, float b) {
+  asm volatile("st.shared.v2.f32 [%0], {%1, %2};" ::"r"(saddr), "f"(a), "f"(b) : "memory");
+}
+__device__ __forceinline__ void stg_v4(void* gptr, uint4 v) {
+  asm volatile("st.global.v4.b32 [%0], {%1, %2, %3, %4};" ::"l"(gptr), "r"(v.x), "r"(v.y), "r"(v.z), "r"(v.w) : "memory");
+}
 __device__ __forceinline__ uint4 lds_v4(uint32_t saddr) {
   uint4 v;
   asm volatile("ld.shared.v4.b32 {%0, %1, %2, %3}, [%4];" : "=r"(v.x), "=r"(v.y), "=r"(v.z), "=r"(v.w) : "r"(saddr) : "memory");
diff --git a/kandinsky-2_b200/csrc/k2_conv_gemm.cu b/kandinsky-2_b200/csrc/k2_conv_gemm.cu
--- a/kandinsky-2_b200/csrc/k2_conv_gemm.cu
+++ b/kandinsky-2_b200/csrc/k2_conv_gemm.cu
@@ -10,24 +10,22 @@
 constexpr int BM = 128;
 constexpr int BK = 64;
 constexpr int A_STAGE_BYTES = BM * BK * 2;
-constexpr int ACC_PAD = 4;
-
-constexpr int EPI_STAGE_FLOATS = 32 * 33;
-constexpr int EPI_BYTES = 4 * EPI_STAGE_FLOATS * 4 + 4 * 256 * 4;
 constexpr int SMEM_LIMIT = 227 * 1024;
-
-template <int BN, int ES>
+constexpr int BLOCK_BYTES = 16 * 128;
+
+template <int BN>
 struct Cfg {
   static constexpr int B_STAGE_BYTES = BN * BK * 2;
   static constexpr int STAGE_BYTES = A_STAGE_BYTES + B_STAGE_BYTES;
-  static constexpr int BNC = (BN < 64) ? BN : (ES == 2 ? 128 : 64);
-  static_assert(ES == 1 || BN % 128 == 0, "two epilogue sets need N tiles of 128 or 256");
-  static constexpr int ACC_BYTES = BM * (BNC + ACC_PAD) * 4;
+  static constexpr int NP = BN / 64;
+  static constexpr int WARP_STAGING_BYTES = NP * BLOCK_BYTES;
+  static constexpr int STAGING_BYTES = 8 * WARP_STAGING_BYTES;
+  static constexpr int FOLD_BYTES = 8 * NP * 32 * 16;
   static constexpr int BAR_BYTES = 256;
-  static constexpr int FIXED = ACC_BYTES + ES * EPI_BYTES + BAR_BYTES + 1024;
+  static constexpr int FIXED = STAGING_BYTES + FOLD_BYTES + BAR_BYTES + 1024;
   static constexpr int STAGES = (SMEM_LIMIT - FIXED) / STAGE_BYTES > 6 ? 6 : (SMEM_LIMIT - FIXED) / STAGE_BYTES;
   static constexpr int SMEM_BYTES = STAGES * STAGE_BYTES + FIXED;
-  static_assert(STAGES >= 2, "conv_gemm: shared memory does not hold two pipeline stages");
+  static_assert(STAGES >= (BN <= 64 ? 6 : BN == 128 ? 5 : BN == 192 ? 4 : 3), "conv_gemm: N tile lost a pipeline stage");
 };
 
 __device__ __forceinline__ void decode_m_tile(const ConvGemmParams& p, int m_idx, int& n0, int& y0,
@@ -46,307 +44,219 @@
   n0 = tn_i * p.TN;
 }
 
-template <int N>
-__device__ __forceinline__ void acc_ld(const float* src, uint32_t (&r)[N]) {
-#pragma unroll
-  for (int v = 0; v < N / 4; ++v) {
-    const float4 t = *reinterpret_cast<const float4*>(src + 4 * v);
-    r[4 * v] = __float_as_uint(t.x);
-    r[4 * v + 1] = __float_as_uint(t.y);
-    r[4 * v + 2] = __float_as_uint(t.z);
-    r[4 * v + 3] = __float_as_uint(t.w);
-  }
-}
-
-template <int BN, int ES>
-__device__ __forceinline__ void epilogue_tile(const ConvGemmParams& p, const float* acc, int ew, int lane, int n0, int y0,
-                                              int x0, int cbase, int split, int m_idx, float* stat_smem, int es_arg,
-                                              int phase) {
-  const int es = (ES == 1) ? 0 : es_arg;
-  const int row = ew * 32 + lane;
+__device__ __forceinline__ int row_pixel(const ConvGemmParams& p, int row, int n0, int y0, int x0, int phase) {
   const int thw = p.TH * p.TW;
-  constexpr int CH = (BN >= 32) ? 32 : 16;
-  const float* arow = acc + row * (BN + ACC_PAD);
-      const int tn = row / thw;
-      const int rem = row - tn * thw;
-      const int th = rem / p.TW;
-      const int tw = rem - th * p.TW;
-      const int n = n0 + tn, y = y0 + th, x = x0 + tw;
-      const bool valid = (tn < p.TN) && (n < p.NB) && (y < p.H) && (x < p.W);
-      const long long out_row = p.up2 ? (static_cast<long long>(n) * (2 * p.H) + (2 * y + (phase >> 1))) * (2 * p.W) + (2 * x + (phase & 1))
-                                      : (static_cast<long long>(n) * p.H + y) * p.W + x;
-      const int m_in = p.up2 ? m_idx - phase * p.m_tiles_phase : m_idx;
-      auto part_index = [&](long long base) { return p.up2 ? base * 4 + phase : base; };
-      if constexpr (BN % 64 == 0) {
-        if ((p.out_mode == 0 && p.Cout % 64 == 0) || (p.out_mode == 2 && p.Cout % 32 == 0)) {
-          const uint32_t stage = smem_u32(stat_smem + (es * 4 + ew) * EPI_STAGE_FLOATS);
-          float* bsm = stat_smem + 4 * ES * EPI_STAGE_FLOATS + (es * 4 + ew) * 256;
-          const int my_pix = valid ? static_cast<int>(out_row) : -1;
-          const int sub = lane >> 3, piece = lane & 7;
-          int pix[8];
-#pragma unroll
-          for (int i = 0; i < 8; ++i) pix[i] = __shfl_sync(0xffffffffu, my_pix, i * 4 + sub);
-          const uint32_t own = stage + lane * 128;
-          if (p.out_mode == 2) {
-            float* wsb = p.ws + static_cast<long long>(split) * p.M_total * p.Cout;
-#pragma unroll 1
-            for (int j = 0; j < BN / 32; ++j) {
-              const int col0 = cbase + j * 32;
-              if (col0 >= p.Cout) break;
-              if constexpr (ES > 1) {
-                if ((j % ES) != es) continue;
-              }
-              uint32_t r[32];
-              acc_ld(arow + j * 32, r);
-#pragma unroll
-              for (int v = 0; v < 8; ++v)
-                sts_v4(own + ((v ^ (lane & 7)) << 4), r[v * 4], r[v * 4 + 1], r[v * 4 + 2], r[v * 4 + 3]);
-              __syncwarp();
-#pragma unroll
-              for (int i = 0; i < 8; ++i) {
-                const int rr = i * 4 + sub;
-                const uint4 v4 = lds_v4(stage + rr * 128 + ((piece ^ (rr & 7)) << 4));
-                if (pix[i] >= 0)
-                  *reinterpret_cast<uint4*>(wsb + static_cast<long long>(pix[i]) * p.Cout + col0 + piece * 4) = v4;
-              }
-              __syncwarp();
-            }
-            return;
-          }
-          constexpr int NP = BN / 64;
+  const int tn = row / thw;
+  const int rem = row - tn * thw;
+  const int th = rem / p.TW;
+  const int tw = rem - th * p.TW;
+  const int n = n0 + tn, y = y0 + th, x = x0 + tw;
+  if (!((tn < p.TN) && (n < p.NB) && (y < p.H) && (x < p.W))) return -1;
+  return p.up2 ? (n * (2 * p.H) + (2 * y + (phase >> 1))) * (2 * p.W) + (2 * x + (phase & 1)) : (n * p.H + y) * p.W + x;
+}
+
+__device__ __forceinline__ void load_res_block(const ConvGemmParams& p, uint32_t blk, const int (&pix)[4], int c0, int lane) {
+  if (c0 >= p.Cout) return;
+  const int sub = lane >> 3, piece = lane & 7;
+#pragma unroll
+  for (int i = 0; i < 4; ++i) {
+    const int rr = 4 * i + sub;
+    const __half* src = p.residual + (pix[i] >= 0 ? static_cast<long long>(pix[i]) * p.ldr + c0 + piece * 8 : 0);
+    cp_async_16(blk + rr * 128 + ((piece ^ (rr & 7)) << 4), src, pix[i] >= 0 ? 16 : 0);
+  }
+  cp_async_commit();
+}
+
+struct Staged {
+  int pix[4];
+  int cbase;
+  int nblk;
+  int next;
+  int gn_row;
+};
+
+template <int BN>
+__device__ __forceinline__ void stage_tile(const ConvGemmParams& p, const float (&acc)[BN / 2], uint32_t stg, int lane,
+                                           int pixA, int pixB, int cbase) {
+  const int la = lane >> 2;
+  const int cq = 2 * (lane & 3);
+#pragma unroll
+  for (int jb = 0; jb < BN / 64; ++jb) {
+    const int c0 = cbase + 64 * jb;
+    if (c0 < p.Cout) {
+#pragma unroll
+      for (int jj = 0; jj < 8; ++jj) {
+        float2 b = make_float2(0.f, 0.f);
+        if (p.bias) b = make_float2(__ldg(p.bias + c0 + 8 * jj + cq), __ldg(p.bias + c0 + 8 * jj + cq + 1));
+#pragma unroll
+        for (int h = 0; h < 2; ++h) {
+          const int i = 4 * (8 * jb + jj) + 2 * h;
+          float f0 = acc[i], f1 = acc[i + 1];
           if (p.bias) {
-#pragma unroll
-            for (int c = lane; c < BN; c += 32) bsm[c] = (cbase + c < p.Cout) ? __ldg(p.bias + cbase + c) : 0.f;
-            __syncwarp();
-          }
-          __half* outb = reinterpret_cast<__half*>(p.out);
-          float4 st[NP];
-          uint4 rpre[8];
-          auto load_res = [&](int jp) {
-            const int c0 = cbase + jp * 64;
-#pragma unroll
-            for (int i = 0; i < 8; ++i) {
-              rpre[i] = make_uint4(0u, 0u, 0u, 0u);
-              if (pix[i] >= 0 && c0 < p.Cout)
-                rpre[i] = *reinterpret_cast<const uint4*>(p.residual + static_cast<long long>(pix[i]) * p.ldr + c0 + piece * 8);
-            }
-          };
-          if constexpr (ES == 1) {
-            if (p.residual) load_res(0);
-          }
-#pragma unroll
-          for (int jp = 0; jp < NP; ++jp) {
-            const int col0 = cbase + jp * 64;
-            st[jp] = make_float4(0.f, 0.f, 0.f, 0.f);
-            if (col0 < p.Cout && (ES == 1 || (jp % ES) == es)) {
-              if constexpr (ES > 1) {
-                if (p.residual) load_res(jp);
-              }
-              if (p.residual) {
-#pragma unroll
-                for (int i = 0; i < 8; ++i) {
-                  const int rr = i * 4 + sub;
-                  sts_v4(stage + rr * 128 + ((piece ^ (rr & 7)) << 4), rpre[i].x, rpre[i].y, rpre[i].z, rpre[i].w);
-                }
-                __syncwarp();
-              }
-              if constexpr (ES == 1) {
-                if (p.residual && jp + 1 < NP) load_res(jp + 1);
-              }
-#pragma unroll
-              for (int v = 0; v < 8; ++v) {
-                uint32_t r[8];
-                acc_ld(arow + jp * 64 + v * 8, r);
-                float f[8];
-#pragma unroll
-                for (int e = 0; e < 8; ++e) f[e] = __uint_as_float(r[e]);
-                if (p.bias) {
-                  const float4 b0 = *reinterpret_cast<const float4*>(bsm + jp * 64 + v * 8);
-                  const float4 b1 = *reinterpret_cast<const float4*>(bsm + jp * 64 + v * 8 + 4);
-                  f[0] += b0.x; f[1] += b0.y; f[2] += b0.z; f[3] += b0.w;
-                  f[4] += b1.x; f[5] += b1.y; f[6] += b1.z; f[7] += b1.w;
-                }
-                const uint32_t slot = own + ((v ^ (lane & 7)) << 4);
-                if (p.residual) {
-                  const uint4 rv = lds_v4(slot);
-                  const __half2* rh = reinterpret_cast<const __half2*>(&rv);
-#pragma unroll
-                  for (int e = 0; e < 4; ++e) {
-                    const float2 t = __half22float2(rh[e]);
-                    f[2 * e] += t.x;
-                    f[2 * e + 1] += t.y;
-                  }
-                }
-                uint32_t o[4];
-#pragma unroll
-                for (int e = 0; e < 4; ++e) {
-                  const __half2 hh = __floats2half2_rn(f[2 * e], f[2 * e + 1]);
-                  o[e] = valid ? *reinterpret_cast<const uint32_t*>(&hh) : 0u;
-                }
-                sts_v4(slot, o[0], o[1], o[2], o[3]);
-              }
-              __syncwarp();
-#pragma unroll
-              for (int i = 0; i < 8; ++i) {
-                const int rr = i * 4 + sub;
-                const uint4 v4 = lds_v4(stage + rr * 128 + ((piece ^ (rr & 7)) << 4));
-                if (pix[i] >= 0)
-                  *reinterpret_cast<uint4*>(outb + static_cast<long long>(pix[i]) * p.ldo + col0 + piece * 8) = v4;
-              }
-              if (p.gn_part) {
-                float4 h0 = make_float4(0.f, 0.f, 0.f, 0.f), h1 = make_float4(0.f, 0.f, 0.f, 0.f);
-#pragma unroll
-                for (int rr = 0; rr < 32; ++rr) {
-                  const uint32_t w = lds_u32(stage + rr * 128 + (((lane >> 2) ^ (rr & 7)) << 4) + ((lane & 3) << 2));
-                  const float2 t = __half22float2(*reinterpret_cast<const __half2*>(&w));
-                  float4& hacc = (rr < 16) ? h0 : h1;
-                  hacc.x += t.x;
-                  hacc.y = fmaf(t.x, t.x, hacc.y);
-                  hacc.z += t.y;
-                  hacc.w = fmaf(t.y, t.y, hacc.w);
-                }
-                if (p.gn_mode == 2) {
-                  const int per = p.tiles_h * p.tiles_w;
-                  const int sp = m_in % per;
-                  const int img = n0 + 2 * ew;
-                  if (2 * ew < p.TN && img < p.NB)
-                    *reinterpret_cast<float4*>(p.gn_part + part_index(static_cast<long long>(img) * per + sp) * p.Cout + col0 + 2 * lane) = h0;
-                  if (2 * ew + 1 < p.TN && img + 1 < p.NB)
-                    *reinterpret_cast<float4*>(p.gn_part + part_index(static_cast<long long>(img + 1) * per + sp) * p.Cout + col0 + 2 * lane) = h1;
-                } else {
-                  st[jp] = make_float4(h0.x + h1.x, h0.y + h1.y, h0.z + h1.z, h0.w + h1.w);
-                }
-              }
-              __syncwarp();
-            }
-          }
-          if (p.gn_part && p.gn_mode == 1) {
-            if constexpr (ES == 1) {
-              float4* mine = reinterpret_cast<float4*>(stat_smem + ew * EPI_STAGE_FLOATS);
-#pragma unroll
-              for (int jp = 0; jp < NP; ++jp) mine[jp * 32 + lane] = st[jp];
-              named_bar_sync(1, 128);
-              if (ew < NP) {
-                const int col0 = cbase + ew * 64;
-                if (col0 < p.Cout) {
-                  float4 acc = make_float4(0.f, 0.f, 0.f, 0.f);
-#pragma unroll
-                  for (int w = 0; w < 4; ++w) {
-                    const float4 t = reinterpret_cast<const float4*>(stat_smem + w * EPI_STAGE_FLOATS)[ew * 32 + lane];
-                    acc.x += t.x; acc.y += t.y; acc.z += t.z; acc.w += t.w;
-                  }
-                  *reinterpret_cast<float4*>(p.gn_part + part_index(m_in) * p.Cout + col0 + 2 * lane) = acc;
-                }
-              }
-              named_bar_sync(1, 128);
-            } else {
-              float4* mine = reinterpret_cast<float4*>(stat_smem + (es * 4 + ew) * EPI_STAGE_FLOATS);
-#pragma unroll
-              for (int jp = 0; jp < NP; ++jp) mine[jp * 32 + lane] = st[jp];
-              named_bar_sync(1 + es, 128);
-              const int jp_f = es + ew * ES;
-              if (jp_f < NP) {
-                const int col0 = cbase + jp_f * 64;
-                if (col0 < p.Cout) {
-                  float4 acc = make_float4(0.f, 0.f, 0.f, 0.f);
-#pragma unroll
-                  for (int w = 0; w < 4; ++w) {
-                    const float4 t =
-                        reinterpret_cast<const float4*>(stat_smem + (es * 4 + w) * EPI_STAGE_FLOATS)[jp_f * 32 + lane];
-                    acc.x += t.x; acc.y += t.y; acc.z += t.z; acc.w += t.w;
-                  }
-                  *reinterpret_cast<float4*>(p.gn_part + part_index(m_in) * p.Cout + col0 + 2 * lane) = acc;
-                }
-              }
-              named_bar_sync(1 + es, 128);
-            }
-          }
-          return;
-        }
-      }
-#pragma unroll 1
-      for (int j = 0; j < BN / CH; ++j) {
-        uint32_t r[CH];
-        acc_ld(arow + j * CH, r);
-        const int col0 = cbase + j * CH;
-        if (valid && col0 < p.Cout) {
-          if (p.out_mode == 2) {
-            float* w = p.ws + (static_cast<long long>(split) * p.M_total + out_row) * p.Cout + col0;
-            if (col0 + CH <= p.Cout) {
-#pragma unroll
-              for (int v = 0; v < CH / 4; ++v)
-                *reinterpret_cast<uint4*>(w + v * 4) = make_uint4(r[v * 4], r[v * 4 + 1], r[v * 4 + 2], r[v * 4 + 3]);
-            } else {
-#pragma unroll
-              for (int e = 0; e < CH; ++e)
-                if (col0 + e < p.Cout) w[e] = __uint_as_float(r[e]);
-            }
-          } else if (p.out_mode == 0) {
-            __half* orow = reinterpret_cast<__half*>(p.out) + out_row * p.ldo + col0;
-            const __half* rrow = p.residual ? p.residual + out_row * p.ldr + col0 : nullptr;
-            if (col0 + CH <= p.Cout) {
-#pragma unroll
-              for (int v = 0; v < CH / 8; ++v) {
-                float f[8];
-#pragma unroll
-                for (int e = 0; e < 8; ++e) {
-                  f[e] = __uint_as_float(r[v * 8 + e]);
-                  if (p.bias) f[e] += __ldg(p.bias + col0 + v * 8 + e);
-                }
-                if (rrow) {
-                  uint4 rv = *reinterpret_cast<const uint4*>(rrow + v * 8);
-                  const __half2* rh = reinterpret_cast<const __half2*>(&rv);
-#pragma unroll
-                  for (int e = 0; e < 4; ++e) {
-                    float2 t = __half22float2(rh[e]);
-                    f[2 * e] += t.x;
-                    f[2 * e + 1] += t.y;
-                  }
-                }
-                uint4 ov;
-                __half2* oh = reinterpret_cast<__half2*>(&ov);
-#pragma unroll
-                for (int e = 0; e < 4; ++e) oh[e] = __floats2half2_rn(f[2 * e], f[2 * e + 1]);
-                *reinterpret_cast<uint4*>(orow + v * 8) = ov;
-              }
-            } else {
-#pragma unroll
-              for (int e = 0; e < CH; ++e) {
-                if (col0 + e < p.Cout) {
-                  float f = __uint_as_float(r[e]);
-                  if (p.bias) f += __ldg(p.bias + col0 + e);
-                  if (rrow) f += __half2float(rrow[e]);
-                  orow[e] = __float2half_rn(f);
-                }
-              }
-            }
-          } else {
-            float* o = reinterpret_cast<float*>(p.out);
-#pragma unroll
-            for (int e = 0; e < CH; ++e) {
-              if (col0 + e < p.Cout) {
-                float f = __uint_as_float(r[e]);
-                if (p.bias) f += __ldg(p.bias + col0 + e);
-                o[((static_cast<long long>(n) * p.Cout + (col0 + e)) * p.H + y) * p.W + x] = f;
-              }
-            }
-          }
-        }
-      }
-}
-
-
-template <int BN, int ES>
+            f0 += b.x;
+            f1 += b.y;
+          }
+          const uint32_t slot = stg + jb * BLOCK_BYTES + (la + 8 * h) * 128 + ((jj ^ la) << 4) + (lane & 3) * 4;
+          if (p.residual) {
+            const uint32_t rw = lds_u32(slot);
+            const float2 t = __half22float2(*reinterpret_cast<const __half2*>(&rw));
+            f0 += t.x;
+            f1 += t.y;
+          }
+          const __half2 hh = __floats2half2_rn(f0, f1);
+          const bool valid = (h ? pixB : pixA) >= 0;
+          sts_u32(slot, valid ? *reinterpret_cast<const uint32_t*>(&hh) : 0u);
+        }
+      }
+    }
+  }
+}
+
+template <int BN>
+__device__ __forceinline__ void drain_block(const ConvGemmParams& p, uint32_t stg, Staged& sd, int kw, int lane,
+                                            uint32_t fold) {
+  constexpr int NP = BN / 64;
+  const int jb = sd.next;
+  const uint32_t blk = stg + jb * BLOCK_BYTES;
+  const int col0 = sd.cbase + 64 * jb;
+  const int sub = lane >> 3, piece = lane & 7;
+  __half* outb = reinterpret_cast<__half*>(p.out);
+#pragma unroll
+  for (int i = 0; i < 4; ++i) {
+    const int rr = 4 * i + sub;
+    const uint4 v = lds_v4(blk + rr * 128 + ((piece ^ (rr & 7)) << 4));
+    if (sd.pix[i] >= 0)
+      stg_v4(outb + static_cast<long long>(sd.pix[i]) * p.ldo + col0 + piece * 8, v);
+  }
+  if (p.gn_part) {
+    float4 hs = make_float4(0.f, 0.f, 0.f, 0.f);
+#pragma unroll
+    for (int rr = 0; rr < 16; ++rr) {
+      const uint32_t wv = lds_u32(blk + rr * 128 + (((lane >> 2) ^ (rr & 7)) << 4) + ((lane & 3) << 2));
+      const float2 t = __half22float2(*reinterpret_cast<const __half2*>(&wv));
+      hs.x += t.x;
+      hs.y = fmaf(t.x, t.x, hs.y);
+      hs.z += t.y;
+      hs.w = fmaf(t.y, t.y, hs.w);
+    }
+    if (p.gn_mode == 2) {
+      if (sd.gn_row >= 0)
+        *reinterpret_cast<float4*>(p.gn_part + static_cast<long long>(sd.gn_row) * p.Cout + col0 + 2 * lane) = hs;
+    } else {
+      sts_v4(fold + ((kw * NP + jb) * 32 + lane) * 16, __float_as_uint(hs.x), __float_as_uint(hs.y), __float_as_uint(hs.z),
+             __float_as_uint(hs.w));
+    }
+  }
+  if (++sd.next == sd.nblk && p.gn_part && p.gn_mode == 1) {
+    named_bar_sync(1, 256);
+    if (kw < sd.nblk) {
+      float4 a = make_float4(0.f, 0.f, 0.f, 0.f);
+#pragma unroll
+      for (int e = 0; e < 4; ++e) {
+        const uint4 u = lds_v4(fold + (((2 * e) * NP + kw) * 32 + lane) * 16);
+        const uint4 v = lds_v4(fold + (((2 * e + 1) * NP + kw) * 32 + lane) * 16);
+        a.x += __uint_as_float(u.x) + __uint_as_float(v.x);
+        a.y += __uint_as_float(u.y) + __uint_as_float(v.y);
+        a.z += __uint_as_float(u.z) + __uint_as_float(v.z);
+        a.w += __uint_as_float(u.w) + __uint_as_float(v.w);
+      }
+      *reinterpret_cast<float4*>(p.gn_part + static_cast<long long>(sd.gn_row) * p.Cout + sd.cbase + 64 * kw + 2 * lane) = a;
+    }
+    named_bar_sync(1, 256);
+  }
+}
+
+template <int BN>
+__device__ __forceinline__ void store_partials(const ConvGemmParams& p, const float (&acc)[BN / 2], uint32_t stg, int lane,
+                                               const int (&pix)[4], int cbase, int split) {
+  const int la = lane >> 2, sub = lane >> 3, piece = lane & 7;
+  float* wsb = p.ws + static_cast<long long>(split) * p.M_total * p.Cout;
+#pragma unroll
+  for (int j = 0; j < BN / 32; ++j) {
+    const int col0 = cbase + 32 * j;
+    if (col0 < p.Cout) {
+#pragma unroll
+      for (int jj = 0; jj < 4; ++jj) {
+#pragma unroll
+        for (int h = 0; h < 2; ++h) {
+          const int i = 4 * (4 * j + jj) + 2 * h;
+          const int r = la + 8 * h;
+          const int q = 2 * jj + ((lane & 3) >> 1);
+          sts_v2f(stg + r * 128 + ((q ^ (r & 7)) << 4) + ((lane & 1) << 3), acc[i], acc[i + 1]);
+        }
+      }
+      __syncwarp();
+#pragma unroll
+      for (int i = 0; i < 4; ++i) {
+        const int rr = 4 * i + sub;
+        const uint4 v = lds_v4(stg + rr * 128 + ((piece ^ (rr & 7)) << 4));
+        if (pix[i] >= 0) stg_v4(wsb + static_cast<long long>(pix[i]) * p.Cout + col0 + piece * 4, v);
+      }
+      __syncwarp();
+    }
+  }
+}
+
+template <int BN>
+__device__ __forceinline__ void store_fragments(const ConvGemmParams& p, const float (&acc)[BN / 2], int kw, int lane, int n0,
+                                                int y0, int x0, int phase, int cbase, int split) {
+  const int thw = p.TH * p.TW;
+#pragma unroll
+  for (int h = 0; h < 2; ++h) {
+    const int row = 16 * kw + (lane >> 2) + 8 * h;
+    const int tn = row / thw;
+    const int rem = row - tn * thw;
+    const int th = rem / p.TW;
+    const int tw = rem - th * p.TW;
+    const int n = n0 + tn, y = y0 + th, x = x0 + tw;
+    if (!((tn < p.TN) && (n < p.NB) && (y < p.H) && (x < p.W))) continue;
+    const long long out_row = p.up2 ? (static_cast<long long>(n) * (2 * p.H) + (2 * y + (phase >> 1))) * (2 * p.W) + (2 * x + (phase & 1))
+                                    : (static_cast<long long>(n) * p.H + y) * p.W + x;
+#pragma unroll
+    for (int j = 0; j < BN / 8; ++j) {
+      const int c = cbase + 8 * j + 2 * (lane & 3);
+      const int i = 4 * j + 2 * h;
+      if (c >= p.Cout) continue;
+      if (p.out_mode == 2) {
+        float* wp = p.ws + (static_cast<long long>(split) * p.M_total + out_row) * p.Cout + c;
+        if (c + 1 < p.Cout) *reinterpret_cast<float2*>(wp) = make_float2(acc[i], acc[i + 1]);
+        else wp[0] = acc[i];
+      } else if (p.out_mode == 0) {
+        __half* o = reinterpret_cast<__half*>(p.out) + out_row * p.ldo;
+#pragma unroll
+        for (int e = 0; e < 2; ++e) {
+          if (c + e < p.Cout) {
+            float f = acc[i + e];
+            if (p.bias) f += __ldg(p.bias + c + e);
+            if (p.residual) f += __half2float(p.residual[out_row * p.ldr + c + e]);
+            o[c + e] = __float2half_rn(f);
+          }
+        }
+      } else {
+        float* o = reinterpret_cast<float*>(p.out);
+#pragma unroll
+        for (int e = 0; e < 2; ++e) {
+          if (c + e < p.Cout) {
+            float f = acc[i + e];
+            if (p.bias) f += __ldg(p.bias + c + e);
+            o[((static_cast<long long>(n) * p.Cout + (c + e)) * p.H + y) * p.W + x] = f;
+          }
+        }
+      }
+    }
+  }
+}
+
+template <int BN>
 __global__ void __launch_bounds__(384, 1) conv_gemm_kernel(const __grid_constant__ ConvGemmParams p) {
-  using C = Cfg<BN, ES>;
-  constexpr int BNC = C::BNC;
+  using C = Cfg<BN>;
+  constexpr int NP = C::NP;
   constexpr int NA = BN / 2;
   extern __shared__ uint8_t smem_raw[];
   uint8_t* smem = reinterpret_cast<uint8_t*>((reinterpret_cast<uintptr_t>(smem_raw) + 1023) &
                                              ~static_cast<uintptr_t>(1023));
-  float* acc_smem = reinterpret_cast<float*>(smem + C::STAGES * C::STAGE_BYTES);
-  float* stat_smem = reinterpret_cast<float*>(smem + C::STAGES * C::STAGE_BYTES + C::ACC_BYTES);
-  uint64_t* full_bar = reinterpret_cast<uint64_t*>(smem + C::STAGES * C::STAGE_BYTES + C::ACC_BYTES + ES * EPI_BYTES);
+  uint8_t* staging = smem + C::STAGES * C::STAGE_BYTES;
+  uint64_t* full_bar = reinterpret_cast<uint64_t*>(staging + C::STAGING_BYTES + C::FOLD_BYTES);
   uint64_t* empty_bar = full_bar + C::STAGES;
 
   const int warp_idx = threadIdx.x >> 5;
@@ -418,7 +328,13 @@
   } else {
     setmaxnreg_inc<232>();
     const int g = wg - 1;
-    const int w = warp_idx & 3;
+    const int kw = warp_idx - 4;
+    const uint32_t stg = smem_u32(staging) + kw * C::WARP_STAGING_BYTES;
+    const uint32_t fold = smem_u32(staging + C::STAGING_BYTES);
+    const bool staged_epi = NP > 0 && p.out_mode == 0 && p.Cout % 64 == 0;
+    Staged sd;
+    sd.nblk = 0;
+    sd.next = 0;
     int stage = 0;
     uint32_t phase = 0;
     for (int tile = blockIdx.x; tile < total_tiles; tile += gridDim.x) {
@@ -426,6 +342,27 @@
       const int m_idx = (tile / p.n_tiles) % p.m_tiles;
       const int split = tile / (p.m_tiles * p.n_tiles);
       const int nk = min(p.num_k_chunks, (split + 1) * p.k_per_split) - split * p.k_per_split;
+      const int cbase = n_idx * BN;
+      const bool res_pre = staged_epi && p.residual != nullptr;
+      int rpix[4];
+      {
+        int n0, y0, x0, mphase;
+        decode_m_tile(p, m_idx, n0, y0, x0, mphase);
+#pragma unroll
+        for (int i = 0; i < 4; ++i) rpix[i] = row_pixel(p, 16 * kw + 4 * i + (lane >> 3), n0, y0, x0, mphase);
+      }
+      auto drain_next = [&]() {
+        const int jb = sd.next;
+        drain_block<BN>(p, stg, sd, kw, lane, fold);
+        if (res_pre) {
+          __syncwarp();
+          load_res_block(p, stg + jb * BLOCK_BYTES, rpix, cbase + 64 * jb, lane);
+        }
+      };
+      if (res_pre) {
+        for (int jb = 0; jb < NP; ++jb)
+          if (jb < sd.next || jb >= sd.nblk) load_res_block(p, stg + jb * BLOCK_BYTES, rpix, cbase + 64 * jb, lane);
+      }
       float acc[NA];
 #pragma unroll
       for (int i = 0; i < NA; ++i) acc[i] = 0.f;
@@ -455,37 +392,62 @@
         wgmma_commit();
         wgmma_wait<1>();
         if (prev_stage >= 0 && lane == 0) mbar_arrive(&empty_bar[prev_stage]);
+        if constexpr (NP > 0) {
+          if (sd.next < sd.nblk) drain_next();
+        }
         prev_stage = stage;
         if (++stage == C::STAGES) {
           stage = 0;
           phase ^= 1;
         }
       }
+
+      int n0, y0, x0, mphase;
+      decode_m_tile(p, m_idx, n0, y0, x0, mphase);
+      if constexpr (NP > 0) {
+        if (staged_epi) {
+          while (sd.next < sd.nblk) drain_next();
+          const int pixA = row_pixel(p, 16 * kw + (lane >> 2), n0, y0, x0, mphase);
+          const int pixB = row_pixel(p, 16 * kw + (lane >> 2) + 8, n0, y0, x0, mphase);
+          wgmma_wait<0>();
+          if (prev_stage >= 0 && lane == 0) mbar_arrive(&empty_bar[prev_stage]);
+          if (res_pre) cp_async_wait<0>();
+          __syncwarp();
+          stage_tile<BN>(p, acc, stg, lane, pixA, pixB, cbase);
+          __syncwarp();
+#pragma unroll
+          for (int i = 0; i < 4; ++i) sd.pix[i] = rpix[i];
+          sd.cbase = cbase;
+          sd.nblk = min(NP, (p.Cout - cbase) / 64);
+          sd.next = 0;
+          const int m_in = p.up2 ? m_idx - mphase * p.m_tiles_phase : m_idx;
+          if (p.gn_mode == 2) {
+            const int per = p.tiles_h * p.tiles_w;
+            const int img = n0 + kw;
+            const int part = img * per + m_in % per;
+            sd.gn_row = (kw < p.TN && img < p.NB) ? (p.up2 ? part * 4 + mphase : part) : -1;
+          } else {
+            sd.gn_row = p.up2 ? m_in * 4 + mphase : m_in;
+          }
+          continue;
+        }
+      }
       wgmma_wait<0>();
       if (prev_stage >= 0 && lane == 0) mbar_arrive(&empty_bar[prev_stage]);
-
-      int n0, y0, x0, mphase;
-      decode_m_tile(p, m_idx, n0, y0, x0, mphase);
-      const int r0 = 64 * g + 16 * w + (lane >> 2);
-      const int cq = 2 * (lane & 3);
-#pragma unroll
-      for (int pass = 0; pass < BN / BNC; ++pass) {
-        named_bar_sync(3, 256);
-#pragma unroll
-        for (int i = 0; i < NA; i += 2) {
-          if ((8 * (i >> 2)) / BNC != pass) continue;
-          const int row = r0 + 8 * ((i >> 1) & 1);
-          const int col = 8 * (i >> 2) - pass * BNC + cq;
-          *reinterpret_cast<float2*>(acc_smem + row * (BNC + ACC_PAD) + col) = make_float2(acc[i], acc[i + 1]);
-        }
-        named_bar_sync(3, 256);
-        if (ES == 2 || g == 0)
-          epilogue_tile<BNC, ES>(p, acc_smem, w, lane, n0, y0, x0, n_idx * BN + pass * BNC, split, m_idx, stat_smem, g,
-                                 mphase);
-      }
-    }
-  }
-}
+      if constexpr (NP > 0) {
+        if (p.out_mode == 2 && p.Cout % 32 == 0) {
+          store_partials<BN>(p, acc, stg, lane, rpix, cbase, split);
+          continue;
+        }
+      }
+      store_fragments<BN>(p, acc, kw, lane, n0, y0, x0, mphase, cbase, split);
+    }
+    if constexpr (NP > 0) {
+      while (sd.next < sd.nblk) drain_block<BN>(p, stg, sd, kw, lane, fold);
+    }
+  }
+}
+
 
 __global__ void __launch_bounds__(256) splitk_finalize_kernel(const float* __restrict__ ws, int splits, long long M,
                                                               int Cout, const float* __restrict__ bias,
@@ -558,18 +520,17 @@
 }
 
 
-template <int BN, int ES>
+template <int BN>
 int launch_bn(const ConvGemmParams& p, cudaStream_t stream) {
-  using C = Cfg<BN, ES>;
+  using C = Cfg<BN>;
   static bool attr_set = false;
   if (!attr_set) {
-    K2_CHECK_CUDA(cudaFuncSetAttribute(conv_gemm_kernel<BN, ES>, cudaFuncAttributeMaxDynamicSharedMemorySize,
-                                       C::SMEM_BYTES));
+    K2_CHECK_CUDA(cudaFuncSetAttribute(conv_gemm_kernel<BN>, cudaFuncAttributeMaxDynamicSharedMemorySize, C::SMEM_BYTES));
     attr_set = true;
   }
   int total = p.m_tiles * p.n_tiles * p.splits;
   int grid = total < num_sms() ? total : num_sms();
-  K2_CHECK_CUDA(launch_k(conv_gemm_kernel<BN, ES>, dim3(grid), dim3(384), C::SMEM_BYTES, stream, p));
+  K2_CHECK_CUDA(launch_k(conv_gemm_kernel<BN>, dim3(grid), dim3(384), C::SMEM_BYTES, stream, p));
   return 0;
 }
 
@@ -583,20 +544,13 @@
   return 0;
 }
 
-int launch_conv_gemm(const ConvGemmParams& p, int BN, int epilogue_sets, cudaStream_t stream) {
-  if (epilogue_sets == 2) {
-    switch (BN) {
-      case 128: return launch_bn<128, 2>(p, stream);
-      case 256: return launch_bn<256, 2>(p, stream);
-      default: break;
-    }
-  }
+int launch_conv_gemm(const ConvGemmParams& p, int BN, cudaStream_t stream) {
   switch (BN) {
-    case 16: return launch_bn<16, 1>(p, stream);
-    case 64: return launch_bn<64, 1>(p, stream);
-    case 128: return launch_bn<128, 1>(p, stream);
-    case 192: return launch_bn<192, 1>(p, stream);
-    case 256: return launch_bn<256, 1>(p, stream);
+    case 16: return launch_bn<16>(p, stream);
+    case 64: return launch_bn<64>(p, stream);
+    case 128: return launch_bn<128>(p, stream);
+    case 192: return launch_bn<192>(p, stream);
+    case 256: return launch_bn<256>(p, stream);
     default: return fail("conv_gemm: unsupported BN");
   }
 }
diff --git a/kandinsky-2_b200/csrc/k2_internal.h b/kandinsky-2_b200/csrc/k2_internal.h
--- a/kandinsky-2_b200/csrc/k2_internal.h
+++ b/kandinsky-2_b200/csrc/k2_internal.h
@@ -74,7 +74,7 @@
   int up2;
   int m_tiles_phase;
 };
-int launch_conv_gemm(const ConvGemmParams& p, int BN, int epilogue_sets, cudaStream_t stream);
+int launch_conv_gemm(const ConvGemmParams& p, int BN, cudaStream_t stream);
 int launch_splitk_finalize(const float* ws, int splits, long long M, int Cout, const float* bias, const __half* residual,
                            int ldr, __half* out, int ldo, float2* gn_part, cudaStream_t stream);
 
diff --git a/kandinsky-2_b200/kandinsky2/launch_plan.py b/kandinsky-2_b200/kandinsky2/launch_plan.py
--- a/kandinsky-2_b200/kandinsky2/launch_plan.py
+++ b/kandinsky-2_b200/kandinsky2/launch_plan.py
@@ -25,8 +25,7 @@
     best = None
     if cout > 64:
         bns = [bn0] if splits > 1 else [bn for bn in (128, 192, 256) if bn - 64 < cout or bn == bn0]
-        cands = [(bn0, 0, splits, 1)] + [(bn, 0, splits, es) for bn in bns for es in ((1,) if bn == 192 else (1, 2))
-                                        if (bn, es) != (bn0, 1)]
+        cands = [(bn0, 0, splits, 1)] + [(bn, 0, splits, 1) for bn in bns if bn != bn0]
         if 0 < m_rows <= TUNE_SMALL_M and splits == 1:
             for bn in (128, 192, 256):
                 if bn - 64 >= cout:
diff --git a/profiles/conv_layers.py b/profiles/conv_layers.py
--- a/profiles/conv_layers.py
+++ b/profiles/conv_layers.py
@@ -89,9 +89,13 @@
     ap.add_argument("--min-ms", type=float, default=50.0, help="timed window per configuration")
     ap.add_argument("--mma-n", default="tile", choices=["tile", "64"],
                     help="wgmma N of the build: one instruction per N tile, or m64n64k16 per 64 columns")
+    ap.add_argument("--lib", default=None, help="libk2b200.so to time (default: the in-tree build)")
     args = ap.parse_args()
     if not torch.cuda.is_available():
         raise SystemExit("needs a CUDA sm_90 device")
+    from kandinsky2 import _native
+    if args.lib:
+        _native.LIB_PATH = os.path.abspath(args.lib)
     import bench
     from kandinsky2 import launch_plan, ops
     from kandinsky2.model.gaussian_diffusion import FusedStep, create_ddpm_v22
@@ -99,7 +103,7 @@
     torch.cuda.set_device(dev)
     ops.set_tuning(4, 1)
     res = {"card": _card(), "torch": torch.__version__, "geometry": f"cfg-2: UNet batch {2 * B}, {H}x{W} latents",
-           "mma_n": args.mma_n, "min_ms": args.min_ms}
+           "mma_n": args.mma_n, "min_ms": args.min_ms, "lib": _native.LIB_PATH}
 
     counts = {}
     tune = launch_plan.tune
@@ -133,12 +137,11 @@
         info = [0] * 7
         picked = launch_plan._tune_cache.get((dev.index, launch_plan.TUNE_SMALL_M) + key)
         run(picked, info)
-        picked_cfg = [info[0], 0, info[2], (picked[3] if picked and picked[3] else 1)]
+        picked_cfg = [info[0], 0, info[2], 1]
         cout = shp["N"]
         cfgs = []
         if cout > 64:
-            cfgs = [(bn, 0, 1, es) for bn in (128, 192, 256) if bn - 64 < cout or bn == info[0]
-                    for es in ((1,) if bn == 192 else (1, 2))]
+            cfgs = [(bn, 0, 1, 1) for bn in (128, 192, 256) if bn - 64 < cout or bn == info[0]]
         if tuple(picked_cfg) not in cfgs:
             cfgs.append(tuple(picked_cfg))
         rows = []
@@ -153,16 +156,14 @@
             m_tiles = info[3] * (4 if "up2" in shp["desc"] else 1)
             chunks = m_tiles * ((cout + bn - 1) // bn) * (shp["K"] // 64)
             l2_bytes = chunks * (16384 + bn * 128)
-            rows.append(dict(n_tile=bn, epilogue_sets=cfg[3], splits=splits, ms=round(ms, 5), reps=reps,
+            rows.append(dict(n_tile=bn, splits=splits, ms=round(ms, 5), reps=reps,
                              tflops=round(flops / (ms * 1e-3) / 1e12, 1),
                              smem_operand_bytes_per_flop=round(smem_bpf, 5),
                              l2_operand_bytes_per_flop=round(l2_bytes / flops, 5),
                              l2_operand_TBps=round(l2_bytes / (ms * 1e-3) / 1e12, 2)))
-        pick = next((r for r in rows if [r["n_tile"], r["splits"], r["epilogue_sets"]] ==
-                     [picked_cfg[0], picked_cfg[2], picked_cfg[3]]), rows[0])
+        pick = next((r for r in rows if [r["n_tile"], r["splits"]] == [picked_cfg[0], picked_cfg[2]]), rows[0])
         layers.append(dict(shape=shp["desc"], key=repr(key), launches_per_step=n, gemm_gflop=round(2e-9 * shp["M"] * cout * shp["K"], 3),
-                           picked=dict(n_tile=picked_cfg[0], splits=picked_cfg[2], epilogue_sets=picked_cfg[3],
-                                       tuned=picked is not None),
+                           picked=dict(n_tile=picked_cfg[0], splits=picked_cfg[2], tuned=picked is not None),
                            picked_ms=pick["ms"], configs=rows))
     total = sum(l["launches_per_step"] * l["picked_ms"] for l in layers)
     for l in layers:
@@ -171,15 +172,14 @@
     res["conv_ms_per_step_at_picked"] = round(total, 3)
     res["layers"] = layers
 
-    print(f"# {res['card']}  (mma_n={args.mma_n})  conv time per step at the picked configurations: {total:.2f} ms")
-    print(f"{'shape':44s} {'n':>2s} {'share':>6s} {'pick':>9s}  " + "  ".join(f"{c:>9s}" for c in
-          ("128/1", "128/2", "192/1", "256/1", "256/2")) + "   (TFLOP/s at N tile / epilogue sets, splits 1)")
+    print(f"# {res['card']}  {res['lib']}  (mma_n={args.mma_n})  conv time per step at the picked configurations: {total:.2f} ms")
+    print(f"{'shape':44s} {'n':>2s} {'share':>6s} {'pick':>7s}  " + "  ".join(f"{c:>7d}" for c in (128, 192, 256))
+          + "   (TFLOP/s at N tile, splits 1)")
     for l in layers:
-        by = {(r["n_tile"], r["epilogue_sets"]): r["tflops"] for r in l["configs"] if r["splits"] == 1}
+        by = {r["n_tile"]: r["tflops"] for r in l["configs"] if r["splits"] == 1}
         pk = l["picked"]
         print(f"{l['shape'][:44]:44s} {l['launches_per_step']:2d} {100 * l['share_of_conv_time']:5.1f}% "
-              f"{pk['n_tile']:>3d}/{pk['epilogue_sets']}/{pk['splits']:<3d}  " +
-              "  ".join(f"{by.get(c, float('nan')):9.1f}" for c in ((128, 1), (128, 2), (192, 1), (256, 1), (256, 2))))
+              f"{pk['n_tile']:>3d}/{pk['splits']:<3d}  " + "  ".join(f"{by.get(c, float('nan')):7.1f}" for c in (128, 192, 256)))
     if args.out:
         os.makedirs(os.path.dirname(os.path.abspath(args.out)), exist_ok=True)
         with open(args.out, "w") as f:
```

Result: faster. 31.81, median of 6 (+2.9%).
